# violetamenendez/zest-nerf

Measured on AMD Instinct MI355X. Metric: rendered rays/sec (1024-ray x 128-sample batch per GPU), higher is better.
Workload: dtype bf16; 1 GPU; nsff_static_1024x128; rays_per_gpu=1024, samples_per_ray=128, rays_total=1024, collective=none, ranks=1, backend=none

## Files before the change

### zest-nerf_amd/csrc/fused.cuh

```cuda
#pragma once
#include "mlp_engine.cuh"
#include "zest_sample_ops.cuh"

namespace zest {

constexpr int kMaxViews = 16;
constexpr int kCamStride = 24;

struct FusedNet {
    const float *bias;
    const uint4 *tiles;
    const float4 *vol;
    const float4 *imgs;
    const float *w2cs, *intr;
    int D, Hv, Wv, V, H, W;
    int head, v2;
};

struct FusedArgs {
    const float *ndc, *pts, *z, *dir;
    int R, S;
    FusedNet st, dy;
    float frame_idx;
    int white_bkgd;
    int bpr;
    float *partials;
    float *out;
    unsigned long long *stamps;
    int ray_ranges;
};

struct RayState {
    float Ts = 1.f, Tb = 1.f, Tf = 1.f;
    float s[5] = {0, 0, 0, 0, 0}, bl[5] = {0, 0, 0, 0, 0}, fg[4] = {0, 0, 0, 0};
    __device__ __forceinline__ void chain(const float *p, bool dyn) {
#pragma unroll
        for (int i = 0; i < 5; i++) s[i] += Ts * p[1 + i];
        Ts *= p[0];
        if (dyn) {
#pragma unroll
            for (int i = 0; i < 5; i++) bl[i] += Tb * p[7 + i];
            Tb *= p[6];
#pragma unroll
            for (int i = 0; i < 4; i++) fg[i] += Tf * p[13 + i];
            Tf *= p[12];
        }
    }
    __device__ __forceinline__ void emit(int white_bkgd, float *__restrict__ out_row) const {
        float4 *o = reinterpret_cast<float4 *>(out_row);
        const float bg = white_bkgd ? 1.0f - s[4] : 0.0f;
        o[0] = make_float4(s[0] + bg, s[1] + bg, s[2] + bg, s[3]);
        o[1] = make_float4(s[4], bl[0], bl[1], bl[2]);
        o[2] = make_float4(bl[3], fg[0], fg[1], fg[2]);
        float zero = 0.f;
        asm volatile("" : "+v"(zero));
        o[3] = make_float4(fg[3], bl[4], zero, zero);
    }
    __device__ __forceinline__ void save(float *c) const {
        c[0] = Ts, c[1] = Tb, c[2] = Tf;
#pragma unroll
        for (int i = 0; i < 5; i++) c[3 + i] = s[i], c[8 + i] = bl[i];
#pragma unroll
        for (int i = 0; i < 4; i++) c[13 + i] = fg[i];
    }
    __device__ __forceinline__ void load(const float *c) {
        Ts = c[0], Tb = c[1], Tf = c[2];
#pragma unroll
        for (int i = 0; i < 5; i++) s[i] = c[3 + i], bl[i] = c[8 + i];
#pragma unroll
        for (int i = 0; i < 4; i++) fg[i] = c[13 + i];
    }
};
constexpr int kCarryFloats = 20;

template <class Rec>
__device__ __forceinline__ void combine_ray(Rec rec, int bpr, bool dyn, int white_bkgd, float *__restrict__ out_row) {
    RayState st;
    for (int b = 0; b < bpr; b++) st.chain(rec(b), dyn);
    st.emit(white_bkgd, out_row);
}

template <int EP, int C, int L, int NK>
__device__ __forceinline__ void encode_pe_operand(const float (&x)[4], int grp, OpArr<NK, ep_parts(EP)> &op) {
    static_assert((L / 2) * C + 1 <= NK * 8 && L % 2 == 0, "position layout");
    const float quarter = (grp & 1) ? 0.25f : 0.0f;
    const float gscale = (grp & 2) ? 2.0f * 0.15915494309189535f : 0.15915494309189535f;
    const float gband = (grp & 2) ? 2.0f : 1.0f;
    float rev[C];
#pragma unroll
    for (int c = 0; c < C; c++) rev[c] = x[c] * gscale;
    const float raw = grp == 0 ? x[0] : (grp == 1 ? x[1] : (grp == 2 ? x[2] : (C > 3 ? x[3] : 0.0f)));
#pragma unroll
    for (int t = 0; t < NK; t++) {
        float v[8];
#pragma unroll
        for (int e = 0; e < 8; e++) {
            const int m = 8 * t + e;
            if (m < (L / 2) * C) {
                if constexpr (EP == ZEST_PREC_F16X3) {
                    float sn, cs;
                    zest_sincos(x[m % C] * (gband * (float)(1 << (2 * (m / C)))), &sn, &cs);
                    v[e] = (grp & 1) ? cs : sn;
                } else {
                    const float r = fmaf(rev[m % C], (float)(1 << (2 * (m / C))), quarter);
                    v[e] = __builtin_amdgcn_sinf(__builtin_amdgcn_fractf(r));
                }
            } else if (m == (L / 2) * C) {
                v[e] = raw;
            } else {
                v[e] = 0.0f;
            }
        }
        store_tile<EP>(v, op, t);
    }
}

__device__ __forceinline__ float4 zest_color_tap_fast(const float4 *__restrict__ img, int H, int W,
                                                      const float *__restrict__ P, float px, float py, float pz) {
    const float4 r0 = *reinterpret_cast<const float4 *>(P), r1 = *reinterpret_cast<const float4 *>(P + 4),
                 r2 = *reinterpret_cast<const float4 *>(P + 8);
    const float qx = fmaf(pz, r0.z, fmaf(py, r0.y, fmaf(px, r0.x, r0.w)));
    const float qy = fmaf(pz, r1.z, fmaf(py, r1.y, fmaf(px, r1.x, r1.w)));
    const float qz = fmaf(pz, r2.z, fmaf(py, r2.y, fmaf(px, r2.x, r2.w)));
    const float rz = __builtin_amdgcn_rcpf(qz);
    float fx = qx * rz, fy = qy * rz;
    const float wm = (float)(W - 1), hm = (float)(H - 1);
    const float mask = (fx > 0.0f && fx < wm && fy > 0.0f && fy < hm) ? 1.0f : 0.0f;
    fx = fminf(fmaxf(fx, 0.0f), wm), fy = fminf(fmaxf(fy, 0.0f), hm);
    const float x0f = floorf(fx), y0f = floorf(fy);
    const float tx = fx - x0f, ty = fy - y0f;
    const int x0 = (int)x0f, y0 = (int)y0f;
    const int i00 = y0 * W + x0, dx = x0 + 1 < W ? 1 : 0, dy = y0 + 1 < H ? W : 0;
#ifdef ZEST_EXPERIMENT_TAP_SAME
    const float4 a = img[i00 & 0], b = img[(i00 + dx) & 0], d = img[(i00 + dy) & 0], e = img[(i00 + dy + dx) & 0];
#else
    const float4 a = img[i00], b = img[i00 + dx], d = img[i00 + dy], e = img[i00 + dy + dx];
#endif
    const float w00 = (1.0f - tx) * (1.0f - ty), w10 = tx * (1.0f - ty), w01 = (1.0f - tx) * ty, w11 = tx * ty;
    float4 o;
    o.x = fmaf(w11, e.x, fmaf(w01, d.x, fmaf(w10, b.x, w00 * a.x)));
    o.y = fmaf(w11, e.y, fmaf(w01, d.y, fmaf(w10, b.y, w00 * a.y)));
    o.z = fmaf(w11, e.z, fmaf(w01, d.z, fmaf(w10, b.z, w00 * a.z)));
    o.w = mask;
    return o;
}

template <int EP, int NK>
__device__ __forceinline__ void encode_feat_operand(const FusedNet &n, const float *cams_lds,
                                                    const float (&ndc)[4], const float (&pw)[3],
                                                    int grp, bool valid, OpArr<NK, ep_parts(EP)> &op) {
    float v[NK * 8];
#pragma unroll
    for (int i = 0; i < NK * 8; i++) v[i] = 0.0f;
    auto view_tap = [&](int view, float *dst) {
        const int vc = view < n.V ? view : n.V - 1;
        const float *cl = cams_lds + vc * kCamStride;
        float4 o;
        if constexpr (EP == ZEST_PREC_F16X3) {
            ZestCam cam;
#pragma unroll
            for (int i = 0; i < 3; i++) {
#pragma unroll
                for (int j = 0; j < 4; j++) cam.r[i][j] = cl[4 * i + j];
#pragma unroll
                for (int j = 0; j < 3; j++) cam.k[i][j] = cl[12 + 3 * i + j];
            }
#ifdef ZEST_EXPERIMENT_TAP_SAME
            o = zest_color_tap<true>(n.imgs, n.H, n.W, cam, pw[0], pw[1], pw[2]);
#else
            o = zest_color_tap(n.imgs + (size_t)vc * n.H * n.W, n.H, n.W, cam, pw[0], pw[1], pw[2]);
#endif
        } else {
            o = zest_color_tap_fast(n.imgs + vc * (n.H * n.W), n.H, n.W, cl, pw[0], pw[1], pw[2]);
        }
        const bool on = view < n.V;
        dst[0] = on ? o.x : 0.f, dst[1] = on ? o.y : 0.f, dst[2] = on ? o.z : 0.f, dst[3] = on ? o.w : 0.f;
    };
#ifdef ZEST_EXPERIMENT_NO_GATHER
    valid = false;
#endif
#ifdef ZEST_EXPERIMENT_FAKE_FEAT
    if (valid) {
#pragma unroll
        for (int i = 0; i < NK * 8; i++)
            v[i] = __builtin_amdgcn_fractf(ndc[0] * (13.37f + (float)i) + ndc[2] * 7.1f + (float)grp * 0.31f) - 0.25f;
    }
    valid = false;
#endif
    const int rv = feat_volume_round(n.V);
    if (valid) {
        float vv[4] = {0.f, 0.f, 0.f, 0.f};
        if (grp < 2) {
            float fx = zest_unnorm(ndc[0], n.Wv), fy = zest_unnorm(ndc[1], n.Hv), fz = zest_unnorm(ndc[2], n.D);
            fx = fminf(fmaxf(fx, -2.0f), (float)n.Wv + 1.0f);
            fy = fminf(fmaxf(fy, -2.0f), (float)n.Hv + 1.0f);
            fz = fminf(fmaxf(fz, -2.0f), (float)n.D + 1.0f);
            const float x0f = floorf(fx), y0f = floorf(fy), z0f = floorf(fz);
            const float tx = fx - x0f, ty = fy - y0f, tz = fz - z0f;
            const int x0 = (int)x0f, y0 = (int)y0f, z0 = (int)z0f;
            float4 tap[8];
            float wgt[8];
#pragma unroll
            for (int c = 0; c < 8; c++) {
                const int dx = c & 1, dy = (c >> 1) & 1, dz = c >> 2;
                const int xi = x0 + dx, yi = y0 + dy, zi = z0 + dz;
                const bool ok = (unsigned)xi < (unsigned)n.Wv && (unsigned)yi < (unsigned)n.Hv &&
                                (unsigned)zi < (unsigned)n.D;
                const int xc = min(max(xi, 0), n.Wv - 1), yc = min(max(yi, 0), n.Hv - 1),
                          zc = min(max(zi, 0), n.D - 1);
                wgt[c] = ok ? (dx ? tx : 1.0f - tx) * (dy ? ty : 1.0f - ty) * (dz ? tz : 1.0f - tz) : 0.0f;
#ifdef ZEST_EXPERIMENT_TAP_SAME
                tap[c] = n.vol[(((yc * n.Wv + xc) * n.D + zc) & 0) + grp];
#else
                tap[c] = n.vol[2 * ((yc * n.Wv + xc) * n.D + zc) + grp];
#endif
            }
#pragma unroll
            for (int c = 0; c < 8; c++) {
                vv[0] = fmaf(wgt[c], tap[c].x, vv[0]), vv[1] = fmaf(wgt[c], tap[c].y, vv[1]);
                vv[2] = fmaf(wgt[c], tap[c].z, vv[2]), vv[3] = fmaf(wgt[c], tap[c].w, vv[3]);
            }
        }
#pragma unroll
        for (int r = 0; r < 2 * NK; r++) {
            float *dst = v + 8 * (r >> 1) + 4 * (r & 1);
            if (r < rv) {
                view_tap(4 * r + grp, dst);
            } else if (r == rv) {
                if (n.V > 4 * rv) view_tap(grp >= 2 ? 4 * rv + grp - 2 : n.V, dst);
                if (grp < 2) dst[0] = vv[0], dst[1] = vv[1], dst[2] = vv[2], dst[3] = vv[3];
            }
        }
    }
#pragma unroll
    for (int t = 0; t < NK; t++) {
        float w8[8];
#pragma unroll
        for (int e = 0; e < 8; e++) w8[e] = v[8 * t + e];
        store_tile<EP>(w8, op, t);
    }
}

template <bool PROJ>
__device__ __forceinline__ void stage_cams(const FusedNet &n, float *lds) {
    if (!n.w2cs) return;
    const int nv = n.imgs ? n.V : 1;
    for (int i = threadIdx.x; i < nv * kCamStride; i += blockDim.x) {
        const int v = i / kCamStride, k = i % kCamStride;
        float val = 0.0f;
        if constexpr (PROJ) {
            if (k < 12 && n.intr) {
                const int row = k >> 2, col = k & 3;
                const float *K = n.intr + 9 * v + 3 * row, *Rt = n.w2cs + 16 * v + col;
                val = fmaf(K[2], Rt[8], fmaf(K[1], Rt[4], K[0] * Rt[0]));
            } else if (k >= 12) {
                val = n.w2cs[16 * v + (k - 12)];
            }
        } else {
            if (k < 12) val = n.w2cs[16 * v + k];
            else if (k < 21 && n.intr) val = n.intr[9 * v + (k - 12)];
        }
        lds[i] = val;
    }
}

#ifndef ZEST_FUSED_WAVES
#define ZEST_FUSED_WAVES 8
#endif
constexpr int kFusedWaves = ZEST_FUSED_WAVES;
constexpr int kPartialFloats = 20;
constexpr int fused_cb(int EP) { return EP == ZEST_PREC_F16X3 ? 1 : 2; }

struct BlockSamples {
    float x[4], pw[3], zz, dist;
    bool valid;
};

template <int BS>
__device__ __forceinline__ float block_sum(float v) {
    if constexpr (BS == 32) return lower_half_sum(v);
    v += dpp_f<0xB1>(0.f, v);
    v += dpp_f<0x4E>(0.f, v);
    v += dpp_f<0x141>(0.f, v);
    v += dpp_f<0x140>(0.f, v);
    return readlane_f<0>(v);
}
template <int BS>
__device__ __forceinline__ float block_excl_prod(float f, int c, float *total) {
    if constexpr (BS == 32) return lower_half_excl_prod(f, c, total);
    float v = f;
    v *= dpp_f<0x111>(1.f, v);
    v *= dpp_f<0x112>(1.f, v);
    v *= dpp_f<0x114>(1.f, v);
    v *= dpp_f<0x118>(1.f, v);
    *total = readlane_f<15>(v);
    const float ex = dpp_f<0x138>(1.f, v);
    return c == 0 ? 1.0f : ex;
}

#ifndef ZEST_FUSED_WG_PER_CU
#define ZEST_FUSED_WG_PER_CU 1
#endif
#ifndef ZEST_REBUILD_PTS
#define ZEST_REBUILD_PTS 0
#endif
#ifndef ZEST_GATHER_FENCE
#define ZEST_GATHER_FENCE 1
#endif
#ifndef ZEST_EARLY_DYN_GATHER
#define ZEST_EARLY_DYN_GATHER 0
#endif
template <int EP, int NT_FEAT_S, bool DYN, int NT_FEAT_D, bool V2S = false>
__global__ __launch_bounds__(kFusedWaves * 64, kFusedWaves * ZEST_FUSED_WG_PER_CU / 4) void fused_blocks_kernel(FusedArgs a) {
    constexpr bool MOD_S = NT_FEAT_S > 0, MOD_D = NT_FEAT_D > 0;
    constexpr int NP = ep_parts(EP), CB = fused_cb(EP), BS = 16 * CB;
    if constexpr (EP == ZEST_PREC_F16) engine_fp16_overflow_clamp();
    constexpr int UNITS_S = stream_units(4, NT_FEAT_S, NP), UNITS_D = DYN ? stream_units(6, NT_FEAT_D, NP) : 0;
    using Ring = RingTiles<kFusedWaves, UNITS_S, UNITS_D>;
    constexpr int kFdBytes = (DYN && MOD_D && ZEST_EARLY_DYN_GATHER) ? kFusedWaves * CB * (NT_FEAT_D / 2) * NP * 1024 : 0;
    constexpr int kStBytes = DYN ? kFusedWaves * 32 * 24 : 0;
    constexpr bool kMc = mcache_for(EP, MOD_S, NT_FEAT_S / 2) || (DYN && mcache_for(EP, MOD_D, NT_FEAT_D / 2));
    constexpr int kMcWaveBytes = kMc ? kMcJB * CB * 1024 : 0;
    __shared__ __attribute__((aligned(16))) char lds[kRingUnits * 1024 + 2 * kMaxViews * kCamStride * 4 +
                                                     kFusedWaves * 32 * 8 + 2 * kSlots * 4 +
                                                     kFusedWaves * kPartialFloats * 4 + kFusedWaves * 32 * 16 +
                                                     kFdBytes + kStBytes + 2 * kCarryFloats * 4 +
                                                     kFusedWaves * kMcWaveBytes];
    static_assert(sizeof(lds) <= 163840, "LDS budget of one workgroup per CU");
    static_assert((sizeof(lds) - kFusedWaves * kMcWaveBytes) % 16 == 0, "the modulation cache starts 16-byte aligned");
    float *cams_s = reinterpret_cast<float *>(lds + kRingUnits * 1024), *cams_d = cams_s + kMaxViews * kCamStride;
    float2 *zd_lds = reinterpret_cast<float2 *>(cams_d + kMaxViews * kCamStride);
    constexpr bool PROJ = EP != ZEST_PREC_F16X3;
    stage_cams<PROJ>(a.st, cams_s);
    if (DYN) stage_cams<PROJ>(a.dy, cams_d);
    int *ring_flags = reinterpret_cast<int *>(zd_lds + kFusedWaves * 32);
    float *rec_lds = reinterpret_cast<float *>(ring_flags + 2 * kSlots);
    float4 *x_lds = reinterpret_cast<float4 *>(rec_lds + kFusedWaves * kPartialFloats);
    uint4 *fd_lds = reinterpret_cast<uint4 *>(x_lds + kFusedWaves * 32);
    float2 *st_lds = reinterpret_cast<float2 *>(reinterpret_cast<char *>(fd_lds) + kFdBytes);
    float *carry_lds = reinterpret_cast<float *>(reinterpret_cast<char *>(st_lds) + kStBytes);
    char *mc_lds = lds + sizeof(lds) - kFusedWaves * kMcWaveBytes;
#ifdef ZEST_RING_FLAGS
    Ring::init_flags(ring_flags);
#endif
    __syncthreads();

    const int lane0 = threadIdx.x & 63;
    const int wave = __builtin_amdgcn_readfirstlane(threadIdx.x >> 6);
    const Ring tiles{lds, (gptr_u4)a.st.tiles, (gptr_u4)a.dy.tiles, lane0, lane0 >> 4, wave,
                     (unsigned)(wave * Ring::kPieces * 64 + lane0) * 16u,
                     (unsigned)(uintptr_t)(__attribute__((address_space(3))) char *)lds +
                         (unsigned)wave * Ring::kPieces * 1024u
#ifdef ZEST_RING_FLAGS
                     , (unsigned)(uintptr_t)(__attribute__((address_space(3))) char *)ring_flags
#endif
    };
    tiles.init_addr();
    if constexpr (kMc)
        tiles.init_mcache((unsigned)(uintptr_t)(__attribute__((address_space(3))) char *)mc_lds +
                          (unsigned)wave * kMcWaveBytes + (unsigned)lane0 * 16u);
    tiles.prologue();

    const bool ranges = a.ray_ranges != 0;
    const int n_wg = (int)gridDim.x;
#ifndef ZEST_NO_XCD_ORDER
    const int wg = n_wg % 8 == 0 ? (int)(blockIdx.x % 8) * (n_wg / 8) + (int)(blockIdx.x / 8) : (int)blockIdx.x;
#else
    const int wg = (int)blockIdx.x;
#endif
    int range_b0, range_nb;
    if (ranges) {
        range_b0 = (int)((long long)wg * a.R / n_wg) * a.bpr;
        range_nb = (int)((long long)(wg + 1) * a.R / n_wg) * a.bpr - range_b0;
    } else {
        const int n_blocks = a.R * a.bpr;
        const int share = ((n_blocks + kFusedWaves - 1) / kFusedWaves + n_wg - 1) / n_wg * kFusedWaves;
        range_b0 = wg * share, range_nb = min(share, n_blocks - range_b0);
    }
    auto block_of = [&](int pass) {
        const int lb = pass * kFusedWaves + wave;
        return __builtin_amdgcn_readfirstlane(lb < range_nb ? range_b0 + lb : -1);
    };
    auto fetch = [&](int g, int cb, int col, BlockSamples &b) {
        const int r = g >= 0 ? g / a.bpr : 0, s = (g >= 0 ? g % a.bpr : 0) * BS + 16 * cb + col;
        b.valid = g >= 0 && s < a.S;
        b.x[0] = b.x[1] = b.x[2] = 0.f, b.x[3] = a.frame_idx;
        b.pw[0] = b.pw[1] = b.pw[2] = 0.f, b.zz = 0.f, b.dist = 0.f;
        const float *dir = a.dir + 3 * r;
        if (b.valid) {
            const size_t m = (size_t)r * a.S + s;
            const float *zr = a.z + (size_t)r * a.S;
            b.x[0] = a.ndc[3 * m], b.x[1] = a.ndc[3 * m + 1], b.x[2] = a.ndc[3 * m + 2];
            if (a.pts) b.pw[0] = a.pts[3 * m], b.pw[1] = a.pts[3 * m + 1], b.pw[2] = a.pts[3 * m + 2];
            b.zz = zr[s];
            const float dnorm = sqrtf(dir[0] * dir[0] + dir[1] * dir[1] + dir[2] * dir[2]);
            b.dist = ((s + 1 < a.S) ? (zr[s + 1] - b.zz) : 1e10f) * dnorm;
        }
    };
    auto join = [](const f32x4 (&t)[CB], int i) {
        if constexpr (CB == 1) {
            return t[0][i];
        } else {
            const auto r = __builtin_amdgcn_permlane16_swap(__float_as_uint(t[0][i]), __float_as_uint(t[CB - 1][i]), false, false);
            return __uint_as_float(r[0]);
        }
    };
#ifdef ZEST_STAMPS
    unsigned long long st_enc = 0, st_eng = 0, st_comp = 0, st_n = 0;
    const unsigned long long st_t0 = __builtin_amdgcn_s_memtime(), st_r0 = __builtin_amdgcn_s_memrealtime();
#define ZEST_STAMP(var) do { const unsigned long long t_ = __builtin_amdgcn_s_memtime(); var += t_ - st_last; st_last = t_; } while (0)
#else
#define ZEST_STAMP(var) do {} while (0)
#endif
    for (int k = 0; k * kFusedWaves < range_nb; k++) {
        const int pass = k;
#ifdef ZEST_STAMPS
        unsigned long long st_last = __builtin_amdgcn_s_memtime();
        st_n++;
#endif
        const int g = block_of(pass);
        if (__builtin_expect(g < 0, 0)) {
            tiles.finish(0, UNITS_S + UNITS_D);
        } else {
        int lane = lane0;
        asm volatile("" : "+v"(lane));
        const int col = lane & 15, grp = lane >> 4, cbs = lane & (BS - 1);
        int unit = 0;
        f32x4 head_s[CB], rgb_s[CB], head_d[CB], rgb_d[CB];
        auto views_of = [&](const FusedNet &n, const float *cams) {
            return [&, cams](OpArr<1, NP> (&views)[CB]) {
                const float *dir = a.dir + 3 * (g >= 0 ? g / a.bpr : 0);
                float dv[4] = {0.f, 0.f, 0.f, 0.f};
                zest_view_dir(dir, n.w2cs ? cams + (PROJ ? 12 : 0) : nullptr, dv);
                encode_pe_operand<EP, 3, 4, 1>(dv, grp, views[0]);
#pragma unroll
                for (int cb = 1; cb < CB; cb++) views[cb] = views[0];
            };
        };
        OpArr<NT_FEAT_S / 2, NP> feat_s[CB];
#pragma unroll
        for (int cb = 0; cb < CB; cb++) {
            BlockSamples b;
            fetch(g, cb, col, b);
            if (grp == 0) {
                zd_lds[wave * 32 + 16 * cb + col] = make_float2(b.zz, b.valid ? b.dist : -1.0f);
                x_lds[wave * 32 + 16 * cb + col] = make_float4(b.x[0], b.x[1], b.x[2], 0.0f);
            }
            if constexpr (MOD_S) encode_feat_operand<EP, NT_FEAT_S / 2>(a.st, cams_s, b.x, b.pw, grp, b.valid, feat_s[cb]);
#if ZEST_GATHER_FENCE
            if constexpr (DYN && NT_FEAT_S >= 4) __builtin_amdgcn_sched_barrier(0);
#endif
            if constexpr (DYN && MOD_D && ZEST_EARLY_DYN_GATHER) {
                OpArr<NT_FEAT_D / 2, NP> fd;
                encode_feat_operand<EP, NT_FEAT_D / 2>(a.dy, cams_d, b.x, b.pw, grp, b.valid, fd);
#pragma unroll
                for (int t = 0; t < NT_FEAT_D / 2; t++)
#pragma unroll
                    for (int pt = 0; pt < NP; pt++)
                        fd_lds[(((wave * CB + cb) * (NT_FEAT_D / 2) + t) * NP + pt) * 64 + lane] =
                            __builtin_bit_cast(uint4, fd.t[pt][t]);
            }
        }
        auto pts_static = [&](OpArr<2, NP> (&o)[CB], int token) __attribute__((always_inline)) {
#pragma unroll
            for (int cb = 0; cb < CB; cb++) {
                int at = wave * 32 + 16 * cb + col;
                asm volatile("" : "+v"(at) : "v"(token));
                const float4 xv = x_lds[at];
                const float x4[4] = {xv.x, xv.y, xv.z, 0.0f};
#ifdef ZEST_EXPERIMENT_NO_ENCODE
#pragma unroll
                for (int t = 0; t < 2; t++) o[cb].t[0][t] = bf16x8{(short)lane, 1, 2, 3, 4, 5, 6, 7};
#else
                encode_pe_operand<EP, 3, 10, 2>(x4, grp, o[cb]);
#endif
            }
        };
        auto pts_dynamic = [&](OpArr<3, NP> (&o)[CB], int token) __attribute__((always_inline)) {
#pragma unroll
            for (int cb = 0; cb < CB; cb++) {
                int at = wave * 32 + 16 * cb + col;
                asm volatile("" : "+v"(at) : "v"(token));
                const float4 xv = x_lds[at];
                const float x4[4] = {xv.x, xv.y, xv.z, a.frame_idx};
                encode_pe_operand<EP, 4, 10, 3>(x4, grp, o[cb]);
            }
        };
        ZEST_STAMP(st_enc);
        if constexpr (ZEST_REBUILD_PTS) {
            engine_forward<EP, CB, 4, MOD_S, NT_FEAT_S, V2S, true>(tiles, unit, pts_static, feat_s,
                                                        views_of(a.st, cams_s), head_s, rgb_s);
        } else {
            OpArr<2, NP> pts_keep[CB];
            pts_static(pts_keep, 0);
            auto pts_copy = [&](OpArr<2, NP> (&o)[CB], int) __attribute__((always_inline)) {
#pragma unroll
                for (int cb = 0; cb < CB; cb++) o[cb] = pts_keep[cb];
            };
            engine_forward<EP, CB, 4, MOD_S, NT_FEAT_S, V2S, true>(tiles, unit, pts_copy, feat_s,
                                                        views_of(a.st, cams_s), head_s, rgb_s);
        }
        ZEST_STAMP(st_eng);
        float rec[kPartialFloats];
#pragma unroll
        for (int i = 0; i < kPartialFloats; i++) rec[i] = 0.f;
        float zz, dist, cr, cg, cb, al_s;
        bool valid;
        {
            const float2 zd = zd_lds[wave * 32 + cbs];
            zz = zd.x, dist = fmaxf(zd.y, 0.0f), valid = zd.y >= 0.0f;
            float sg = join(head_s, 0);
            cr = join(rgb_s, 0), cg = join(rgb_s, 1), cb = join(rgb_s, 2);
            if (V2S) {
                cr = zest_sigmoid(cr), cg = zest_sigmoid(cg), cb = zest_sigmoid(cb), sg = fmaxf(sg, 0.f);
            }
            cr = zest_sigmoid(cr), cg = zest_sigmoid(cg), cb = zest_sigmoid(cb);
            al_s = valid ? 1.0f - expf(-fmaxf(sg, 0.f) * dist) : 0.0f;
            float tot;
            const float w = al_s * block_excl_prod<BS>(1.0f - al_s + 1e-10f, cbs, &tot);
            rec[0] = tot;
            rec[1] = block_sum<BS>(w * cr), rec[2] = block_sum<BS>(w * cg), rec[3] = block_sum<BS>(w * cb);
            rec[4] = block_sum<BS>(w * zz), rec[5] = block_sum<BS>(w);
        }
        if (DYN) {
            const float blend_s = zest_sigmoid(join(head_s, 1));
            if (lane < BS) {
                st_lds[(wave * 3 + 0) * 32 + lane] = make_float2(cr, cg);
                st_lds[(wave * 3 + 1) * 32 + lane] = make_float2(cb, al_s);
                st_lds[(wave * 3 + 2) * 32 + lane] = make_float2(blend_s, 0.0f);
            }
            OpArr<NT_FEAT_D / 2, NP> feat_d[CB];
            if constexpr (MOD_D && ZEST_EARLY_DYN_GATHER) {
#pragma unroll
                for (int cbi = 0; cbi < CB; cbi++)
#pragma unroll
                    for (int t = 0; t < NT_FEAT_D / 2; t++)
#pragma unroll
                        for (int pt = 0; pt < NP; pt++)
                            feat_d[cbi].t[pt][t] = __builtin_bit_cast(
                                bf16x8, fd_lds[(((wave * CB + cbi) * (NT_FEAT_D / 2) + t) * NP + pt) * 64 + lane]);
            } else if constexpr (MOD_D) {
#pragma unroll
                for (int cbi = 0; cbi < CB; cbi++) {
                    BlockSamples b;
                    fetch(g, cbi, col, b);
                    encode_feat_operand<EP, NT_FEAT_D / 2>(a.dy, cams_d, b.x, b.pw, grp, b.valid, feat_d[cbi]);
                }
            }
            ZEST_STAMP(st_comp);
            if constexpr (ZEST_REBUILD_PTS) {
                engine_forward<EP, CB, 6, MOD_D, NT_FEAT_D, false, true>(tiles, unit, pts_dynamic, feat_d,
                                                            views_of(a.dy, cams_d), head_d, rgb_d);
            } else {
                OpArr<3, NP> pts_keep[CB];
                pts_dynamic(pts_keep, 0);
                auto pts_copy = [&](OpArr<3, NP> (&o)[CB], int) __attribute__((always_inline)) {
#pragma unroll
                    for (int cb = 0; cb < CB; cb++) o[cb] = pts_keep[cb];
                };
                engine_forward<EP, CB, 6, MOD_D, NT_FEAT_D, false, true>(tiles, unit, pts_copy, feat_d,
                                                            views_of(a.dy, cams_d), head_d, rgb_d);
            }
            ZEST_STAMP(st_eng);
            const float2 s0 = st_lds[(wave * 3 + 0) * 32 + cbs], s1 = st_lds[(wave * 3 + 1) * 32 + cbs],
                         s2 = st_lds[(wave * 3 + 2) * 32 + cbs];
            cr = s0.x, cg = s0.y, cb = s1.x, al_s = s1.y;
            const float blend = s2.x;
            const float er = zest_sigmoid(join(rgb_d, 0)), eg = zest_sigmoid(join(rgb_d, 1)),
                        eb = zest_sigmoid(join(rgb_d, 2));
            const float sg_d = join(head_d, 0);
            const float a_fg = valid ? 1.0f - expf(-fmaxf(sg_d, 0.f) * dist) : 0.0f;
            const float a_d = a_fg * blend, a_st = al_s * (1.0f - blend);
            float tot_b, tot_f;
            const float Tb = block_excl_prod<BS>((1.0f - a_d) * (1.0f - a_st) + 1e-10f, cbs, &tot_b);
            const float wf = a_fg * block_excl_prod<BS>(1.0f - a_fg + 1e-10f, cbs, &tot_f);
            const float wd = Tb * a_d, ws = Tb * a_st;
            rec[6] = tot_b;
            rec[7] = block_sum<BS>(wd * er + ws * cr), rec[8] = block_sum<BS>(wd * eg + ws * cg);
            rec[9] = block_sum<BS>(wd * eb + ws * cb), rec[10] = block_sum<BS>((wd + ws) * zz);
            rec[11] = block_sum<BS>(wd);
            rec[12] = tot_f;
            rec[13] = block_sum<BS>(wf * er), rec[14] = block_sum<BS>(wf * eg), rec[15] = block_sum<BS>(wf * eb);
            rec[16] = block_sum<BS>(wf * zz);
        }
        if (lane == 0 && g >= 0) {
            float4 *o = ranges ? reinterpret_cast<float4 *>(rec_lds + wave * kPartialFloats)
                               : reinterpret_cast<float4 *>(a.partials + (size_t)g * kPartialFloats);
#pragma unroll
            for (int i = 0; i < (DYN ? 5 : 2); i++)
                o[i] = make_float4(rec[4 * i], rec[4 * i + 1], rec[4 * i + 2], rec[4 * i + 3]);
        }
        }
#ifdef ZEST_EXPERIMENT_NO_FINISH
        if (false) {
#else
        if (ranges) {
#endif
            __syncthreads();
            const int rb = g >= 0 ? g % a.bpr : 0;
            if (lane0 == 0 && g >= 0 && (wave == 0 || rb == 0)) {
                RayState st;
                if (rb != 0) st.load(carry_lds + ((k + 1) & 1) * kCarryFloats);
                const int n = min(a.bpr - rb, kFusedWaves - wave);
                for (int b = 0; b < n; b++) st.chain(rec_lds + (wave + b) * kPartialFloats, DYN);
                if (rb + n == a.bpr) st.emit(a.white_bkgd, a.out + (size_t)(g / a.bpr) * 16);
                else st.save(carry_lds + (k & 1) * kCarryFloats);
            }
        }
        ZEST_STAMP(st_comp);
        tiles.next_pass();
    }
    tiles.drain();
#ifdef ZEST_RING_FLAGS
    if (tiles.poisoned && lane0 == 0) {
        a.partials[0] = __builtin_nanf("");
    }
#endif
#ifdef ZEST_STAMPS
    if (a.stamps && lane0 == 0) {
        unsigned long long *o = a.stamps + (size_t)(blockIdx.x * kFusedWaves + wave) * 8;
        o[0] = __builtin_amdgcn_s_memtime() - st_t0, o[1] = st_enc, o[2] = st_eng, o[3] = st_comp;
        o[4] = tiles.t_wait, o[5] = tiles.t_issue, o[6] = __builtin_amdgcn_s_memrealtime() - st_r0,
        o[7] = st_n | (tiles.t_vm << 16);
    }
#endif
}

#define ZEST_FUSED_VARIANT(ptag, EP, tag, NTS, DYN, NTD, V2S) ZEST_FUSED_VARIANT_(ptag, EP, tag, NTS, DYN, NTD, V2S)
#define ZEST_FUSED_VARIANT_(ptag, EP, tag, NTS, DYN, NTD, V2S)                                   \
    int fused_launch_##ptag##_##tag(const FusedArgs &a, int blocks, hipStream_t stream) {        \
        hipLaunchKernelGGL((fused_blocks_kernel<EP, NTS, DYN, NTD, V2S>), dim3(blocks),          \
                           dim3(kFusedWaves * 64), 0, stream, a);                                \
        ZEST_RETURN_LAUNCH("zest_render_fused_fwd(" #ptag "_" #tag ")");                         \
    }                                                                                            \
    int fused_units_##ptag##_##tag(int which) {                                                  \
        return which == 0 ? stream_units(4, NTS, ep_parts(EP)) : (DYN ? stream_units(6, NTD, ep_parts(EP)) : 0); \
    }

#define ZEST_FUSED_DECL1(ptag, tag)                                                     \
    int fused_launch_##ptag##_##tag(const FusedArgs &a, int blocks, hipStream_t stream); \
    int fused_units_##ptag##_##tag(int which);
#define ZEST_FUSED_DECL(tag) ZEST_FUSED_DECL1(bf16, tag) ZEST_FUSED_DECL1(f16, tag) ZEST_FUSED_DECL1(x3, tag)
ZEST_FUSED_DECL(s0)
ZEST_FUSED_DECL(s2)
ZEST_FUSED_DECL(s4)
ZEST_FUSED_DECL(s0d0)
ZEST_FUSED_DECL(s2d0)
ZEST_FUSED_DECL(s4d0)
ZEST_FUSED_DECL(s2d2)
ZEST_FUSED_DECL(s4d2)
ZEST_FUSED_DECL(s2v)
ZEST_FUSED_DECL(s4v)

}
```

### zest-nerf_amd/csrc/fused.hip

```cpp
#include <string.h>
#include "fused.cuh"
#include "mlp_plan.h"

namespace zest {

__global__ void fused_combine_kernel(const float *__restrict__ partials, int R, int bpr, int dyn,
                                     int white_bkgd, float *__restrict__ out) {
    const int r = blockIdx.x * blockDim.x + threadIdx.x;
    if (r >= R) return;
    combine_ray([&](int b) { return partials + ((size_t)r * bpr + b) * kPartialFloats; }, bpr, dyn != 0,
                white_bkgd, out + (size_t)r * 16);
}

}

namespace {

bool fill_net(const zest_mlp_desc *d, const void *packed, const zest_view_set *vs, int pts_ch, int precision,
              zest::FusedNet *n, int *nt_feat, int *units, const char **err) {
    memset(n, 0, sizeof(*n));
    if (!d || !packed) return *err = "descriptor and packed weights are required", false;
    if (d->in_ch_pts != pts_ch) return *err = "unexpected in_ch_pts for this slot", false;
    if (d->net_type != 0 && d->net_type != 2) return *err = "net_type must be 0 ('v0') or 2 ('v2')", false;
    zest::MlpPlan plan;
    if (!zest::build_plan(*d, precision, zest::ORDER_ACC, &plan, err, false)) return false;
    n->bias = (const float *)packed;
    n->tiles = (const uint4 *)((const char *)packed + plan.bias_bytes);
    n->head = d->head, n->v2 = d->net_type == 2;
    *nt_feat = d->use_feat ? plan.nt_feat : 0;
    *units = plan.n_tiles;
    if (((uintptr_t)packed & 15) != 0) return *err = "packed weights must be 16-byte aligned", false;
    if (vs) {
        n->w2cs = vs->w2cs, n->intr = vs->intrinsics;
        n->vol = (const float4 *)vs->vol_cl, n->imgs = (const float4 *)vs->imgs_cl;
        n->D = vs->D, n->Hv = vs->Hv, n->Wv = vs->Wv, n->V = vs->V, n->H = vs->H, n->W = vs->W;
    }
    if (d->use_feat) {
        if (!vs || !vs->vol_cl || !vs->imgs_cl || !vs->w2cs || !vs->intrinsics)
            return *err = "a net with features needs volume, images and cameras", false;
        if (vs->D < 1 || vs->Hv < 1 || vs->Wv < 1 || vs->H < 2 || vs->W < 2)
            return *err = "bad volume / image shape", false;
        if ((long long)vs->D * vs->Hv * vs->Wv >= (1LL << 30))
            return *err = "volume too large for the fused kernel's 32-bit voxel indices (2^30 voxels)", false;
        if (vs->V < 1 || vs->V > zest::kMaxViews || 8 + 4 * vs->V != d->in_ch_feat)
            return *err = "view count does not match in_ch_feat = 8 + 4V", false;
        if (((uintptr_t)vs->vol_cl | (uintptr_t)vs->imgs_cl) & 15)
            return *err = "volume / images must be 16-byte aligned", false;
    } else {
        n->vol = nullptr, n->imgs = nullptr;
    }
    return true;
}

}

#ifdef ZEST_STAMPS
constexpr size_t kStampBytes = 1024 * 8 * 8 * 8;
#else
constexpr size_t kStampBytes = 0;
#endif

static int g_pass_shape = 0;

extern "C" int zest_render_fused_set_passes(int shape) {
    ZEST_CHECK_ARG(shape >= 0 && shape <= 2,
                   "zest_render_fused_set_passes: shape must be 0 (auto), 1 (dense: equal block shares) or 2 (ray ranges)");
    g_pass_shape = shape;
    return 0;
}

extern "C" int zest_render_fused_pass_shape(int R, int S, int precision, int cus, int *ray_ranges, int *n_wg,
                                            int *rounds) {
    ZEST_CHECK_ARG(R >= 0 && S >= 1 && zest::prec_is_engine(precision) && ray_ranges,
                   "zest_render_fused_pass_shape: bad argument");
    if (cus <= 0) {
        int dev = 0;
        if (hipGetDevice(&dev) != hipSuccess ||
            hipDeviceGetAttribute(&cus, hipDeviceAttributeMultiprocessorCount, dev) != hipSuccess)
            cus = 256;
    }
    const int bs = 16 * zest::fused_cb(precision), bpr = (S + bs - 1) / bs;
    const int W = zest::kFusedWaves;
    const int P = zest_div_up((long long)R * bpr, W), G0 = P < cus ? P : cus;
    const int dense_rounds = G0 ? zest_div_up(P, G0) : 0, dense_wg = G0 ? zest_div_up(P, dense_rounds) : 0;
    const int n = R < cus ? R : cus;
    const int range_rounds = n ? zest_div_up((long long)zest_div_up(R, n) * bpr, W) : 0;
    int take = range_rounds <= dense_rounds ? 1 : 0;
    if (g_pass_shape == 1) take = 0;
    if (g_pass_shape == 2) take = 1;
    *ray_ranges = take;
    if (n_wg) *n_wg = take ? n : dense_wg;
    if (rounds) *rounds = take ? range_rounds : dense_rounds;
    return 0;
}

extern "C" size_t zest_render_fused_workspace(int R, int S) {
    if (R <= 0 || S <= 0) return 16 + kStampBytes;
    return (size_t)R * ((S + 15) / 16) * zest::kPartialFloats * sizeof(float) + kStampBytes;
}

extern "C" int zest_render_fused_fwd(const float *ndc, const float *pts, const float *z,
                                     const float *rays_dir, int R, int S,
                                     const zest_mlp_desc *desc_static, const void *packed_static,
                                     const zest_view_set *views_static,
                                     const zest_mlp_desc *desc_dynamic, const void *packed_dynamic,
                                     const zest_view_set *views_dynamic, float frame_idx,
                                     int precision, int white_bkgd, void *workspace, float *out,
                                     void *stream) {
    if (R == 0) return 0;
    ZEST_CHECK_ARG(ndc && z && rays_dir && out && workspace,
                   "zest_render_fused_fwd: ndc, z, rays_dir, workspace, out required");
    ZEST_CHECK_ARG(((uintptr_t)workspace & 15) == 0, "zest_render_fused_fwd: workspace must be 16-byte aligned");
    ZEST_CHECK_ARG(R >= 0 && S >= 1, "zest_render_fused_fwd: bad shape R=%d S=%d", R, S);
    ZEST_CHECK_ARG(zest::prec_is_engine(precision),
                   "zest_render_fused_fwd: precision must be ZEST_PREC_BF16, _F16 or _F16X3 (the exact-product "
                   "fp32 kernel exists per operator only: zest_mlp_fwd)");
    ZEST_CHECK_ARG(((uintptr_t)out & 15) == 0, "zest_render_fused_fwd: out must be 16-byte aligned");
    zest::FusedArgs a;
    memset(&a, 0, sizeof(a));
    a.ndc = ndc, a.pts = pts, a.z = z, a.dir = rays_dir, a.R = R, a.S = S;
    a.frame_idx = frame_idx, a.white_bkgd = white_bkgd, a.out = out;
    const int bs = 16 * zest::fused_cb(precision);
    a.bpr = (S + bs - 1) / bs, a.partials = (float *)workspace;
#ifdef ZEST_STAMPS
    a.stamps = (unsigned long long *)((char *)workspace + zest_render_fused_workspace(R, S) - kStampBytes);
#endif
    const char *err = nullptr;
    int nts = 0, ntd = 0, units_s = 0, units_d = 0;
    ZEST_CHECK_ARG(fill_net(desc_static, packed_static, views_static, 63, precision, &a.st, &nts, &units_s, &err),
                   "zest_render_fused_fwd: static net: %s", err);
    const bool dyn = desc_dynamic != nullptr;
    if (dyn) {
        ZEST_CHECK_ARG(fill_net(desc_dynamic, packed_dynamic, views_dynamic, 84, precision, &a.dy, &ntd, &units_d, &err),
                       "zest_render_fused_fwd: dynamic net: %s", err);
        ZEST_CHECK_ARG(desc_static->head == ZEST_HEAD_BLEND && desc_dynamic->head == ZEST_HEAD_DYNAMIC,
                       "zest_render_fused_fwd: blending needs a static net with the blend head and "
                       "a dynamic net with the scene-flow heads");
    }
    ZEST_CHECK_ARG(pts || (!a.st.vol && !a.dy.vol), "zest_render_fused_fwd: pts required with features");
    if (R == 0) return 0;
    int dev = 0, cus = 256;
    if (hipGetDevice(&dev) != hipSuccess ||
        hipDeviceGetAttribute(&cus, hipDeviceAttributeMultiprocessorCount, dev) != hipSuccess)
        cus = 256;
    int blocks = 0;
    zest_render_fused_pass_shape(R, S, precision, cus, &a.ray_ranges, &blocks, nullptr);
    hipStream_t st = (hipStream_t)stream;
    const bool v2s = a.st.v2 != 0;
    ZEST_CHECK_ARG(!(v2s && (dyn || nts == 0)),
                   "zest_render_fused_fwd: a 'v2' net is rendered by the single-net kernels with features only");
    const int key = (v2s ? 1000 : 0) + (dyn ? 100 : 0) + nts * 10 + ntd;
    int rc = -1;
#define ZEST_CASE1(ptag, tag)                                                                    \
    ZEST_CHECK_ARG(zest::fused_units_##ptag##_##tag(0) == units_s && zest::fused_units_##ptag##_##tag(1) == units_d, \
                   "zest_render_fused_fwd: packed stream is %d+%d units, kernel expects %d+%d",  \
                   units_s, units_d, zest::fused_units_##ptag##_##tag(0), zest::fused_units_##ptag##_##tag(1)); \
    rc = zest::fused_launch_##ptag##_##tag(a, blocks, st);
#define ZEST_CASE(k, tag)                                                                        \
    case k:                                                                                      \
        if (precision == ZEST_PREC_BF16) { ZEST_CASE1(bf16, tag) }                               \
        else if (precision == ZEST_PREC_F16) { ZEST_CASE1(f16, tag) }                            \
        else { ZEST_CASE1(x3, tag) }                                                             \
        break;
    switch (key) {
        ZEST_CASE(0, s0)
        ZEST_CASE(20, s2)
        ZEST_CASE(40, s4)
        ZEST_CASE(100, s0d0)
        ZEST_CASE(120, s2d0)
        ZEST_CASE(140, s4d0)
        ZEST_CASE(122, s2d2)
        ZEST_CASE(142, s4d2)
        ZEST_CASE(1020, s2v)
        ZEST_CASE(1040, s4v)
        default:
            zest_set_error("zest_render_fused_fwd: no fused variant for %d static / %d dynamic feature "
                           "tiles%s", nts, ntd, dyn ? "" : " (static only)");
            return (int)hipErrorInvalidValue;
    }
#undef ZEST_CASE
#undef ZEST_CASE1
    if (rc != 0 || a.ray_ranges) return rc;
    hipLaunchKernelGGL(zest::fused_combine_kernel, dim3(zest_div_up(R, 128)), dim3(128), 0, st,
                       a.partials, R, a.bpr, dyn ? 1 : 0, white_bkgd, out);
    ZEST_RETURN_LAUNCH("zest_render_fused_fwd(combine)");
}
```

### zest-nerf_amd/csrc/mlp.hip

```cpp
#include <string.h>
#include <map>
#include <mutex>
#include <tuple>
#include "mlp_plan.h"
#include "zest_common.cuh"
#include "mlp_engine.cuh"

namespace {

using zest::MlpPlan;

struct DevPlan {
    MlpPlan plan;
    uint32_t *tile_src = nullptr, *bias_src = nullptr, *hdr_src = nullptr;
    uint8_t *unit_part = nullptr;
};

std::mutex g_mu;
std::map<std::tuple<int, int, int, int, int, int, int, int, int, int, int, int>, DevPlan *> g_plans;

constexpr int kOrderBwd = 99;

DevPlan *get_plan(const zest_mlp_desc &d, int precision, int order, bool need_tables) {
    int dev = 0;
    if (hipGetDevice(&dev) != hipSuccess) dev = 0;
    std::lock_guard<std::mutex> lk(g_mu);
    auto key = std::make_tuple(d.in_ch_pts, d.use_feat ? d.in_ch_feat : 0, d.in_ch_views,
                               d.use_feat, d.net_type, d.head, precision, order, d.depth, d.width, d.skip_mask, dev);
    auto it = g_plans.find(key);
    DevPlan *dp = it == g_plans.end() ? nullptr : it->second;
    if (!dp) {
        dp = new DevPlan();
        const char *err = nullptr;
        const bool ok = order == kOrderBwd ? zest::build_bwd_plan(d, &dp->plan, &err)
                                           : zest::build_plan(d, precision, order, &dp->plan, &err);
        if (!ok) {
            zest_set_error("MLP shape not supported: %s", err);
            delete dp;
            return nullptr;
        }
        g_plans[key] = dp;
    }
    if (need_tables && !dp->tile_src) {
        const size_t nt = dp->plan.tile_src.size() * 4, nb = dp->plan.bias_src.size() * 4;
        const size_t nh = dp->plan.hdr_src.size() * 4, np = dp->plan.unit_part.size();
        hipError_t e = hipMalloc(&dp->tile_src, nt);
        if (e == hipSuccess) e = hipMalloc(&dp->unit_part, np ? np : 4);
        if (e == hipSuccess && np) e = hipMemcpy(dp->unit_part, dp->plan.unit_part.data(), np, hipMemcpyHostToDevice);
        if (e == hipSuccess) e = hipMalloc(&dp->bias_src, nb ? nb : 4);
        if (e == hipSuccess) e = hipMalloc(&dp->hdr_src, nh ? nh : 4);
        if (e == hipSuccess) e = hipMemcpy(dp->tile_src, dp->plan.tile_src.data(), nt, hipMemcpyHostToDevice);
        if (e == hipSuccess && nb) e = hipMemcpy(dp->bias_src, dp->plan.bias_src.data(), nb, hipMemcpyHostToDevice);
        if (e == hipSuccess && nh) e = hipMemcpy(dp->hdr_src, dp->plan.hdr_src.data(), nh, hipMemcpyHostToDevice);
        if (e != hipSuccess) {
            zest_set_error("zest_mlp_pack: uploading gather tables: %s", hipGetErrorString(e));
            dp->tile_src = nullptr;
            return nullptr;
        }
    }
    return dp;
}

inline int order_for(int precision) {
    return zest::prec_is_engine(precision) ? zest::ORDER_ACC : zest::ORDER_NATURAL;
}

struct ParamTable {
    const float *p[2 * ZEST_P_COUNT];
};

template <int PREC>
__global__ void pack_kernel(ParamTable pt, const uint32_t *__restrict__ tile_src, size_t n_w,
                            const uint32_t *__restrict__ bias_src, size_t n_b,
                            const uint8_t *__restrict__ unit_part,
                            float *__restrict__ bias_out, void *__restrict__ w_out) {
    const size_t i = (size_t)blockIdx.x * blockDim.x + threadIdx.x;
    if (i < n_b) {
        const uint32_t s = bias_src[i];
        bias_out[i] = s == 0xFFFFFFFFu ? 0.0f : pt.p[2 * (s >> 24) + 1][s & 0xFFFFFF];
    }
    if (i < n_w) {
        const uint32_t s = tile_src[i];
        const float v = s == 0xFFFFFFFFu ? 0.0f : pt.p[2 * (s >> 24)][s & 0xFFFFFF];
        if (PREC == ZEST_PREC_BF16) {
            ((__hip_bfloat16 *)w_out)[i] = __float2bfloat16(v);
        } else if (PREC == ZEST_PREC_F16) {
            ((_Float16 *)w_out)[i] = (_Float16)v;
        } else if (PREC == ZEST_PREC_F16X3) {
            const _Float16 hi = (_Float16)v;
            ((_Float16 *)w_out)[i] = unit_part[i / 512] ? (_Float16)((v - (float)hi) * 2048.0f) : hi;
        } else {
            ((float *)w_out)[i] = v;
        }
    }
}

__global__ void pack_headers_kernel(ParamTable pt, const uint32_t *__restrict__ hdr_src, size_t n,
                                    char *__restrict__ w_out) {
    const size_t i = (size_t)blockIdx.x * blockDim.x + threadIdx.x;
    if (i >= n) return;
    const uint32_t s = hdr_src[i];
    if (s == 0xFFFFFFFFu) return;
    const size_t unit = i / 64, j = i % 64;
    ((float *)(w_out + unit * 1024))[j] = pt.p[2 * (s >> 24) + 1][s & 0xFFFFFF];
}

struct F32Op {
    int njb, nseg, kind0, nt0, kind1, nt1, mod, relu, tile_base, tiles_per_jb, bias_block;
    int src_h, dst;
};
struct F32Prog {
    F32Op op[zest::kNumOps];
    int n_ops, W;
    int P, F, Vw, C_in, C_out, nt_feat, net_v2, act_out, head;
    int rows_pts, rows_feat;
};

constexpr int kF32Samples = 32;

__global__ __launch_bounds__(256, 1) void mlp_f32_kernel(F32Prog pr, const float *__restrict__ bias,
                                                         const float4 *__restrict__ tiles,
                                                         const float *__restrict__ x, int M,
                                                         float *__restrict__ out) {
    extern __shared__ __attribute__((aligned(16))) float smem[];
    float *b_pts = smem;
    float *b_feat = b_pts + pr.rows_pts * 32;
    float *b_views = b_feat + pr.rows_feat * 32;
    float *b_h[2] = {b_views + 32 * 32, b_views + 32 * 32 + pr.W * 32};
    const int tid = threadIdx.x, lane = tid & 63, wave = tid >> 6;
    const int col = lane & 31, half = lane >> 5;
    const int n_in_rows = pr.rows_pts + pr.rows_feat + 32;

    for (int m0 = blockIdx.x * kF32Samples; m0 < M; m0 += gridDim.x * kF32Samples) {
        __syncthreads();
        for (int i = tid; i < n_in_rows * 32; i += 256) smem[i] = 0.0f;
        __syncthreads();
        const int nvalid = min(kF32Samples, M - m0);
        for (int i = tid; i < nvalid * pr.C_in; i += 256) {
            const int s = i / pr.C_in, c = i % pr.C_in;
            const float v = x[(size_t)m0 * pr.C_in + i];
            float *dst = c < pr.P ? b_pts + c * 32
                                  : (c < pr.P + pr.F ? b_feat + (c - pr.P) * 32
                                                     : b_views + (c - pr.P - pr.F) * 32);
            dst[s] = v;
        }
        __syncthreads();
#pragma unroll 1
        for (int o = 0; o < pr.n_ops; o++) {
            const F32Op op = pr.op[o];
            for (int jb = wave; jb < op.njb; jb += 4) {
                const float4 *tp = tiles + ((size_t)op.tile_base + (size_t)jb * op.tiles_per_jb) * 64 + lane;
                f32x16 acc, macc;
                {
                    const float *bb = bias + (size_t)(op.bias_block + jb) * 32 + half * 16;
#pragma unroll
                    for (int i = 0; i < 16; i++) acc[i] = bb[i];
                }
                if (op.mod) {
                    const float *mb = bias + (size_t)jb * 32 + half * 16;
#pragma unroll
                    for (int i = 0; i < 16; i++) macc[i] = mb[i];
                    for (int t = 0; t < pr.nt_feat; t++, tp += 64) {
                        const float4 a = *tp;
                        const float *bp = b_feat + (t * 8 + 4 * half) * 32 + col;
                        macc = __builtin_amdgcn_mfma_f32_32x32x2f32(a.x, bp[0], macc, 0, 0, 0);
                        macc = __builtin_amdgcn_mfma_f32_32x32x2f32(a.y, bp[32], macc, 0, 0, 0);
                        macc = __builtin_amdgcn_mfma_f32_32x32x2f32(a.z, bp[64], macc, 0, 0, 0);
                        macc = __builtin_amdgcn_mfma_f32_32x32x2f32(a.w, bp[96], macc, 0, 0, 0);
                    }
                }
                for (int sg = 0; sg < op.nseg; sg++) {
                    const int kind = sg ? op.kind1 : op.kind0, nt = sg ? op.nt1 : op.nt0;
                    const float *src = kind == zest::SEG_PTS ? b_pts
                                       : kind == zest::SEG_VIEWS ? b_views : b_h[op.src_h];
                    for (int t = 0; t < nt; t++, tp += 64) {
                        const float4 a = *tp;
                        const float *bp = src + (t * 8 + 4 * half) * 32 + col;
                        acc = __builtin_amdgcn_mfma_f32_32x32x2f32(a.x, bp[0], acc, 0, 0, 0);
                        acc = __builtin_amdgcn_mfma_f32_32x32x2f32(a.y, bp[32], acc, 0, 0, 0);
                        acc = __builtin_amdgcn_mfma_f32_32x32x2f32(a.z, bp[64], acc, 0, 0, 0);
                        acc = __builtin_amdgcn_mfma_f32_32x32x2f32(a.w, bp[96], acc, 0, 0, 0);
                    }
                }
#pragma unroll
                for (int i = 0; i < 16; i++) {
                    const int row = 32 * jb + (i & 3) + 8 * (i >> 2) + 4 * half;
                    float v = acc[i];
                    if (op.mod) v = pr.net_v2 ? v + macc[i] : v * macc[i];
                    if (op.relu) v = fmaxf(v, 0.0f);
                    if (op.dst < 2) {
                        b_h[op.dst][row * 32 + col] = v;
                    } else if (col < nvalid) {
                        float *orow = out + (size_t)(m0 + col) * pr.C_out;
                        if (o == pr.n_ops - 1) {
                            if (row < 3) orow[row] = pr.act_out ? zest_sigmoid(v) : v;
                        } else if (row == 0) {
                            orow[3] = pr.act_out ? fmaxf(v, 0.0f) : v;
                        } else if (3 + row < pr.C_out) {
                            const bool is_sf = pr.head == ZEST_HEAD_DYNAMIC && row <= 6;
                            orow[3 + row] = is_sf ? tanhf(v) : zest_sigmoid(v);
                        }
                    }
                }
            }
            __syncthreads();
        }
    }
}

F32Prog make_f32_prog(const MlpPlan &p) {
    F32Prog pr = {};
    const int D = p.shape.D, t = (D - 1) & 1;
    pr.n_ops = p.n_ops, pr.W = p.shape.W;
    for (int o = 0; o < p.n_ops; o++) {
        const zest::OpPlan &s = p.op[o];
        F32Op &d = pr.op[o];
        const int src_h = o < D ? (o + 1) & 1 : (o == D + 2 ? 1 - t : t);
        const int dst = o < D ? o & 1 : (o == D + 1 ? 1 - t : (o == D + 2 ? t : 2));
        d.njb = s.njb, d.nseg = s.nseg, d.kind0 = s.seg[0].kind, d.nt0 = s.seg[0].ntiles;
        d.kind1 = s.seg[1].kind, d.nt1 = s.seg[1].ntiles, d.mod = s.mod, d.relu = s.relu;
        d.tile_base = s.tile_base, d.tiles_per_jb = s.tiles_per_jb, d.bias_block = s.bias_block;
        d.src_h = src_h, d.dst = dst;
    }
    pr.P = p.desc.in_ch_pts, pr.F = p.desc.use_feat ? p.desc.in_ch_feat : 0, pr.Vw = p.desc.in_ch_views;
    pr.C_in = pr.P + pr.F + pr.Vw;
    pr.C_out = p.desc.head == ZEST_HEAD_NONE ? 4 : (p.desc.head == ZEST_HEAD_BLEND ? 5 : 12);
    pr.nt_feat = p.nt_feat, pr.net_v2 = p.desc.net_type >= 2, pr.act_out = p.desc.net_type == 2, pr.head = p.desc.head;
    pr.rows_pts = p.nt_pts * 8, pr.rows_feat = p.nt_feat * 8;
    return pr;
}

}

namespace zest {
size_t bwd_stream_bytes(const zest_mlp_desc &d) {
    DevPlan *dp = get_plan(d, ZEST_PREC_BF16, kOrderBwd, false);
    return dp ? dp->plan.bytes : 0;
}
int bwd_stream_units_of(const zest_mlp_desc &d) {
    DevPlan *dp = get_plan(d, ZEST_PREC_BF16, kOrderBwd, false);
    return dp ? dp->plan.tail_unit0 : -1;
}
int pack_bwd_stream(const zest_mlp_desc &d, const float *const *params, void *packed, hipStream_t stream) {
    DevPlan *dp = get_plan(d, ZEST_PREC_BF16, kOrderBwd, true);
    if (!dp) return (int)hipErrorInvalidValue;
    const MlpPlan &p = dp->plan;
    ParamTable pt;
    for (int i = 0; i < 2 * ZEST_P_COUNT; i++) pt.p[i] = params[i];
    const size_t n_w = p.tile_src.size(), n_h = p.hdr_src.size();
    hipLaunchKernelGGL(pack_kernel<ZEST_PREC_BF16>, dim3(zest_div_up(n_w, 256)), dim3(256), 0, stream, pt, dp->tile_src,
                       n_w, dp->bias_src, (size_t)0, dp->unit_part, (float *)packed, packed);
    hipLaunchKernelGGL(pack_headers_kernel, dim3(zest_div_up(n_h, 256)), dim3(256), 0, stream, pt, dp->hdr_src, n_h,
                       (char *)packed);
    ZEST_RETURN_LAUNCH("zest_mlp_train16_pack");
}
}

extern "C" size_t zest_mlp_packed_bytes(const zest_mlp_desc *desc, int precision) {
    if (!desc) return 0;
    DevPlan *dp = get_plan(*desc, precision, order_for(precision), false);
    return dp ? dp->plan.bytes : 0;
}

extern "C" int zest_mlp_pack(const zest_mlp_desc *desc, int precision, const float *const *params,
                             void *packed, void *stream) {
    ZEST_CHECK_ARG(desc && params && packed, "zest_mlp_pack: null argument");
    DevPlan *dp = get_plan(*desc, precision, order_for(precision), true);
    if (!dp) return (int)hipErrorInvalidValue;
    const MlpPlan &p = dp->plan;
    ParamTable pt;
    for (int i = 0; i < 2 * ZEST_P_COUNT; i++) pt.p[i] = params[i];
    bool need[ZEST_P_COUNT] = {};
    for (int i = 0; i < p.shape.D; i++) need[i] = true;
    need[ZEST_P_PTS_BIAS] = desc->use_feat != 0;
    need[ZEST_P_VIEWS] = need[ZEST_P_FEATURE] = need[ZEST_P_ALPHA] = need[ZEST_P_RGB] = true;
    need[ZEST_P_HEAD0] = desc->head != ZEST_HEAD_NONE;
    need[ZEST_P_HEAD1] = desc->head == ZEST_HEAD_DYNAMIC;
    for (int i = 0; i < ZEST_P_COUNT; i++)
        ZEST_CHECK_ARG(!need[i] || (params[2 * i] && params[2 * i + 1]),
                       "zest_mlp_pack: parameter slot %d (weight and bias) is required", i);
    ZEST_CHECK_ARG(((uintptr_t)packed & 15) == 0, "zest_mlp_pack: packed must be 16-byte aligned");
    const size_t n_w = p.tile_src.size(), n_b = p.bias_src.size();
    const size_t n = n_w > n_b ? n_w : n_b;
    void *w_out = (char *)packed + p.bias_bytes;
#define ZEST_PACK(PREC)                                                                            \
    hipLaunchKernelGGL(pack_kernel<PREC>, dim3(zest_div_up(n, 256)), dim3(256), 0, (hipStream_t)stream, \
                       pt, dp->tile_src, n_w, dp->bias_src, n_b, dp->unit_part, (float *)packed, w_out)
    if (zest::prec_is_engine(precision)) {
        if (precision == ZEST_PREC_BF16) ZEST_PACK(ZEST_PREC_BF16);
        else if (precision == ZEST_PREC_F16) ZEST_PACK(ZEST_PREC_F16);
        else ZEST_PACK(ZEST_PREC_F16X3);
        const size_t n_h = p.hdr_src.size();
        if (n_h)
            hipLaunchKernelGGL(pack_headers_kernel, dim3(zest_div_up(n_h, 256)), dim3(256), 0,
                               (hipStream_t)stream, pt, dp->hdr_src, n_h, (char *)w_out);
    } else {
        ZEST_PACK(ZEST_PREC_F32);
    }
#undef ZEST_PACK
    ZEST_RETURN_LAUNCH("zest_mlp_pack");
}

extern "C" int zest_mlp_fwd(const zest_mlp_desc *desc, int precision, const void *packed,
                            const float *x, int M, float *out, void *stream) {
    if (M == 0) return 0;
    ZEST_CHECK_ARG(desc && packed && x && out, "zest_mlp_fwd: null argument");
    ZEST_CHECK_ARG(M >= 0, "zest_mlp_fwd: M=%d", M);
    DevPlan *dp = get_plan(*desc, precision, order_for(precision), false);
    if (!dp) return (int)hipErrorInvalidValue;
    if (M == 0) return 0;
    const MlpPlan &p = dp->plan;
    const float *bias = (const float *)packed;
    const void *tiles = (const char *)packed + p.bias_bytes;
    if (precision == ZEST_PREC_F32) {
        const F32Prog pr = make_f32_prog(p);
        const size_t lds = (size_t)(pr.rows_pts + pr.rows_feat + 32 + 2 * pr.W) * 32 * sizeof(float);
        const int blocks = zest_div_up(M, kF32Samples);
        hipLaunchKernelGGL(mlp_f32_kernel, dim3(blocks < 4096 ? blocks : 4096), dim3(256), lds,
                           (hipStream_t)stream, pr, bias, (const float4 *)tiles, x, M, out);
        ZEST_RETURN_LAUNCH("zest_mlp_fwd(f32)");
    }
    return zest::mlp_engine_launch(p, tiles, x, M, out, (hipStream_t)stream);
}
```

### zest-nerf_amd/csrc/mlp_engine.cuh

```cuda
#pragma once
#include <hip/hip_bf16.h>
#include "mlp_plan.h"
#include "zest_common.cuh"

typedef __attribute__((ext_vector_type(16))) float f32x16;
typedef __attribute__((ext_vector_type(4))) float f32x4;
typedef __attribute__((ext_vector_type(8))) short bf16x8;
typedef __attribute__((ext_vector_type(4))) float v4f;
typedef __attribute__((ext_vector_type(4))) unsigned v4u;
typedef const __attribute__((address_space(1))) v4u *gptr_u4;
typedef __attribute__((address_space(3))) int lds_int;

namespace zest {

constexpr int stream_units_raw(int nt_pts, int nt_feat, int parts = 1) {
    const int mod = nt_feat * parts, P = nt_pts * parts, H = 16 * parts;
    return 8 * (1 + mod + P) + 6 * 8 * (1 + mod + H) + 8 * (1 + mod + P + H)
           + (1 + H) + 8 * (1 + H) + 4 * (1 + H + 2 * parts) + (1 + H / 2);
}
constexpr int stream_units(int nt_pts, int nt_feat, int parts = 1) {
    return (stream_units_raw(nt_pts, nt_feat, parts) + kStreamAlign - 1) / kStreamAlign * kStreamAlign;
}

#ifndef ZEST_CHUNK
#define ZEST_CHUNK 16
#define ZEST_SLOTS 8
#define ZEST_AHEAD 4
#endif
constexpr int kChunk = ZEST_CHUNK, kSlots = ZEST_SLOTS, kRingUnits = kChunk * kSlots, kAhead = ZEST_AHEAD;
static_assert(kStreamAlign % kRingUnits == 0, "stream padding must be a multiple of the ring size");
static_assert(kSlots >= kAhead + 1, "a slot is refilled while the previous chunk may still be read");

#ifndef ZEST_DEFER_DMA
#define ZEST_DEFER_DMA 0
#endif
#ifndef ZEST_ISSUERS
#define ZEST_ISSUERS 8
#endif
template <int NW, int UNITS_A, int UNITS_B>
struct RingTiles {
    static constexpr int kIssuers = ZEST_ISSUERS < NW ? ZEST_ISSUERS : NW;
    static constexpr int kPieces = kChunk / kIssuers;
    static constexpr int kChunksA = UNITS_A / kChunk, kChunks = (UNITS_A + UNITS_B) / kChunk;
    static_assert(kChunk % kIssuers == 0 && UNITS_A % kRingUnits == 0 && UNITS_B % kRingUnits == 0, "");
    char *ring;
    gptr_u4 src_a, src_b;
    int lane, grp, wave;
    unsigned voff;
    unsigned lds_wave_base;
#ifdef ZEST_RING_FLAGS
    unsigned flags;
    mutable int gen_base = 0;
    mutable int poisoned = 0;
#endif
#ifdef ZEST_STAMPS
    mutable unsigned long long t_wait = 0, t_issue = 0, t_vm = 0;
#endif

    __device__ __forceinline__ void issue(int chunk) const {
        if (kIssuers < NW && wave >= kIssuers) return;
        const int c = chunk % kChunks;
        unsigned off = (unsigned)((c < kChunksA ? c : c - kChunksA) * kChunk * 1024);
        asm volatile("" : "+s"(off));
        const __attribute__((address_space(1))) char *sb =
            (const __attribute__((address_space(1))) char *)(c < kChunksA ? src_a : src_b) + off;
        const unsigned dst = lds_wave_base + (c % kSlots) * kChunk * 1024;
        static_assert(kPieces == 1 || kPieces == 2 || kPieces == 4, "pieces per wave");
        if (kPieces == 1)
            asm volatile("s_mov_b32 m0, %2\n\ts_nop 0\n\tglobal_load_lds_dwordx4 %0, %1"
                         :: "v"(voff), "s"(sb), "s"(dst) : "memory", "m0");
        else if (kPieces == 2)
            asm volatile("s_mov_b32 m0, %2\n\ts_nop 0\n\tglobal_load_lds_dwordx4 %0, %1\n\t"
                         "global_load_lds_dwordx4 %0, %1 offset:1024"
                         :: "v"(voff), "s"(sb), "s"(dst) : "memory", "m0");
        else
            asm volatile("s_mov_b32 m0, %2\n\ts_nop 0\n\tglobal_load_lds_dwordx4 %0, %1\n\t"
                         "global_load_lds_dwordx4 %0, %1 offset:1024\n\t"
                         "global_load_lds_dwordx4 %0, %1 offset:2048\n\t"
                         "global_load_lds_dwordx4 %0, %1 offset:3072"
                         :: "v"(voff), "s"(sb), "s"(dst) : "memory", "m0");
    }
#ifdef ZEST_RING_FLAGS
    static_assert(kSlots >= kAhead + 2, "flag ring: a slot is refilled while laggards read its neighbours");
    static constexpr int off_landed(int slot) { return 8 * (slot % kSlots); }
    static constexpr int off_done(int slot) { return 8 * ((slot % kSlots - kAhead + kSlots) % kSlots) + 4; }
    static __device__ void init_flags(int *f) {
        if (threadIdx.x < 2 * kSlots) f[threadIdx.x] = 0;
        __syncthreads();
        if (threadIdx.x == 0) f[off_done(kSlots - 1) / 4] = -NW;
    }
    template <int OFF_A, int OFF_B>
    __device__ __forceinline__ void bump2() const {
        unsigned long long save;
        asm volatile("s_mov_b64 %0, exec\n\ts_mov_b64 exec, 1\n\t"
                     "ds_add_u32 %2, %1 offset:%3\n\tds_add_u32 %2, %1 offset:%4\n\ts_mov_b64 exec, %0"
                     : "=&s"(save) : "v"(1u), "v"(flags), "i"(OFF_A), "i"(OFF_B) : "memory");
    }
    __device__ __forceinline__ void prologue() const {
#pragma unroll
        for (int c = 0; c < kAhead; c++) issue(c);
        asm volatile("s_waitcnt vmcnt(%0)" ::"i"((kAhead - 1) * kPieces) : "memory");
        unsigned long long save;
        asm volatile("s_mov_b64 %0, exec\n\ts_mov_b64 exec, 1\n\t"
                     "ds_add_u32 %2, %1 offset:%3\n\ts_mov_b64 exec, %0"
                     : "=&s"(save) : "v"(1u), "v"(flags), "i"(off_landed(0)) : "memory");
    }
    __device__ __forceinline__ void next_pass() const { gen_base += kChunks / kSlots; }
    static constexpr int kPreRead = 5;
    typedef int v2i __attribute__((ext_vector_type(2)));
    mutable v2i flag_pre = {0, 0};
    __device__ __forceinline__ void pre_read(int chunk) const {
        flag_pre = *(const volatile __attribute__((address_space(3))) v2i *)(flags + off_landed(chunk));
    }
    template <int OFF>
    __device__ __forceinline__ void await(int need_l, int need_d) const {
        unsigned va = (unsigned)flag_pre.x, vb = (unsigned)flag_pre.y;
        int sa, sb, tries = 1 << 14;
        asm volatile("0:\n\t"
                     "v_readfirstlane_b32 %2, %0\n\t"
                     "v_readfirstlane_b32 %3, %1\n\t"
                     "s_nop 1\n\t"
                     "s_cmp_ge_i32 %2, %6\n\t"
                     "s_cselect_b32 %2, 1, 0\n\t"
                     "s_cmp_ge_i32 %3, %7\n\t"
                     "s_cselect_b32 %3, 1, 0\n\t"
                     "s_and_b32 %2, %2, %3\n\t"
                     "s_cbranch_scc1 1f\n\t"
                     "s_sub_u32 %4, %4, 1\n\t"
                     "s_cmp_eq_u32 %4, 0\n\t"
                     "s_cbranch_scc1 1f\n\t"
                     "s_sleep 1\n\t"
                     "ds_read_b32 %0, %5 offset:%8\n\t"
                     "ds_read_b32 %1, %5 offset:%9\n\t"
                     "s_waitcnt lgkmcnt(0)\n\t"
                     "s_branch 0b\n\t"
                     "1:"
                     : "+v"(va), "+v"(vb), "=&s"(sa), "=&s"(sb), "+s"(tries)
                     : "v"(flags), "s"(need_l), "s"(need_d), "i"(OFF), "i"(OFF + 4)
                     : "memory", "scc");
        if (tries == 0) poisoned = 1;
    }
    __device__ __forceinline__ void enter_chunk(int chunk) const {
#ifdef ZEST_STAMPS
        const unsigned long long t0 = __builtin_amdgcn_s_memtime();
#endif
        asm volatile("s_waitcnt vmcnt(%0)" ::"i"((kAhead - 2) * kPieces) : "memory");
#ifdef ZEST_STAMPS
        t_vm += __builtin_amdgcn_s_memtime() - t0;
#endif
        const int need_l = NW * (gen_base + chunk / kSlots + 1), need_d = NW * (gen_base + (chunk + kAhead) / kSlots);
        if (chunk % kChunks == 0) pre_read(chunk);
        switch (chunk % kSlots) {
#define ZEST_CASE(S) case S: bump2<off_landed(S + 1), off_done(S + kSlots - 1)>(); await<off_landed(S)>(need_l, need_d); break;
            ZEST_CASE(0) ZEST_CASE(1) ZEST_CASE(2) ZEST_CASE(3) ZEST_CASE(4) ZEST_CASE(5) ZEST_CASE(6) ZEST_CASE(7)
            ZEST_CASE(8) ZEST_CASE(9) ZEST_CASE(10) ZEST_CASE(11) ZEST_CASE(12) ZEST_CASE(13) ZEST_CASE(14) ZEST_CASE(15)
#undef ZEST_CASE
        }
        static_assert(kSlots <= 16, "extend the slot switch");
#ifdef ZEST_STAMPS
        const unsigned long long t1 = __builtin_amdgcn_s_memtime();
#endif
        issue(chunk + kAhead);
#ifdef ZEST_STAMPS
        t_wait += t1 - t0, t_issue += __builtin_amdgcn_s_memtime() - t1;
#endif
    }
#else
    __device__ __forceinline__ void prologue() const {
#pragma unroll
        for (int c = 0; c < kAhead; c++) issue(c);
    }
    __device__ __forceinline__ void next_pass() const {}
    __device__ __forceinline__ void enter_chunk(int chunk) const {
#ifdef ZEST_STAMPS
        const unsigned long long t0 = __builtin_amdgcn_s_memtime();
#endif
        flush();
        asm volatile("s_waitcnt vmcnt(%0)" ::"i"((kAhead - 1) * kPieces) : "memory");
#ifdef ZEST_STAMPS
        t_vm += __builtin_amdgcn_s_memtime() - t0;
#endif
#ifndef ZEST_EXPERIMENT_NO_BARRIER
        __builtin_amdgcn_s_barrier();
#endif
        asm volatile("" ::: "memory");
#ifdef ZEST_STAMPS
        const unsigned long long t1 = __builtin_amdgcn_s_memtime();
#endif
#ifndef ZEST_EXPERIMENT_NO_DMA
#if ZEST_DEFER_DMA
        pending = chunk + kAhead;
#else
        issue(chunk + kAhead);
#endif
#endif
#ifdef ZEST_STAMPS
        t_wait += t1 - t0, t_issue += __builtin_amdgcn_s_memtime() - t1;
#endif
    }
#endif
    mutable int pending = -1;
    __device__ __forceinline__ void flush() const {
#if ZEST_DEFER_DMA
#ifdef ZEST_STAMPS
        const unsigned long long t1 = __builtin_amdgcn_s_memtime();
#endif
        if (pending >= 0) issue(pending);
        pending = -1;
#ifdef ZEST_STAMPS
        t_issue += __builtin_amdgcn_s_memtime() - t1;
#endif
#endif
    }
    __device__ __forceinline__ void touch(int unit) const {
        if (unit % kChunk == 0) enter_chunk(unit / kChunk);
#ifdef ZEST_RING_FLAGS
        if (unit % kChunk == kChunk - kPreRead) pre_read(unit / kChunk + 1);
#endif
    }
    mutable unsigned rd_lo = 0, rd_hi = 0, rb_lo = 0, rb_hi = 0;
    mutable unsigned mc = 0;
    __device__ __forceinline__ void init_mcache(unsigned lds_addr) const {
        mc = lds_addr;
        asm volatile("" : "+v"(mc));
    }
    __device__ __forceinline__ void init_addr() const {
        const unsigned base = (unsigned)(uintptr_t)(__attribute__((address_space(3))) char *)ring;
        rd_lo = base + lane * 16, rd_hi = rd_lo + 65536, rb_lo = base + grp * 16, rb_hi = rb_lo + 65536;
        asm volatile("" : "+v"(rd_lo), "+v"(rd_hi), "+v"(rb_lo), "+v"(rb_hi));
    }
    static_assert(kRingUnits <= 128, "two 64 KiB windows");
    template <class T>
    static __device__ __forceinline__ const __attribute__((address_space(3))) T *lds_at(unsigned addr) {
        return (const __attribute__((address_space(3))) T *)(uintptr_t)addr;
    }
    __device__ __forceinline__ bf16x8 load(int unit) const {
        touch(unit);
#ifdef ZEST_EXPERIMENT_NO_LDSREAD
        const int r = unit / kChunk * kChunk % kRingUnits;
#else
        const int r = unit % kRingUnits;
#endif
        const v4u v = *lds_at<v4u>((r < 64 ? rd_lo : rd_hi) + (r % 64) * 1024);
        return *reinterpret_cast<const bf16x8 *>(&v);
    }
    __device__ __forceinline__ f32x4 load_bias(int unit, int which, int rt) const {
        if (which == 0 && rt == 0) touch(unit);
        const int r = unit % kRingUnits;
        return *lds_at<v4f>((r < 64 ? rb_lo : rb_hi) + (r % 64) * 1024 + which * 128 + rt * 64);
    }
    __device__ __forceinline__ void finish(int unit, int end) const {
#pragma unroll
        for (int u = (unit + kChunk - 1) / kChunk * kChunk; u < end; u += kChunk) {
#ifdef ZEST_RING_FLAGS
            pre_read(u / kChunk);
#endif
            enter_chunk(u / kChunk);
        }
        flush();
    }
    __device__ __forceinline__ void drain() const { asm volatile("s_waitcnt vmcnt(0)" ::: "memory"); }
};

constexpr int ep_parts(int EP) { return EP == ZEST_PREC_F16X3 ? 2 : 1; }
constexpr float kLoScale = 2048.0f, kLoUnscale = 1.0f / 2048.0f;

typedef __attribute__((ext_vector_type(2))) float f32x2_t;
typedef __attribute__((ext_vector_type(2))) __bf16 bf16x2_t;
typedef __attribute__((ext_vector_type(2))) _Float16 f16x2_t;
typedef __attribute__((ext_vector_type(8))) _Float16 f16x8_t;

template <int EP>
__device__ __forceinline__ unsigned pack_pair(float lo, float hi) {
    const f32x2_t f = {lo, hi};
    if constexpr (EP == ZEST_PREC_BF16) {
        const bf16x2_t r = __builtin_convertvector(f, bf16x2_t);
        return __builtin_bit_cast(unsigned, r);
    } else {
        const f16x2_t r = __builtin_convertvector(f, f16x2_t);
        return __builtin_bit_cast(unsigned, r);
    }
}
__device__ __forceinline__ unsigned pack_bf16(float lo, float hi) { return pack_pair<ZEST_PREC_BF16>(lo, hi); }

__device__ __forceinline__ void split_pair(float a, float b, unsigned &hi, unsigned &lo) {
    const f32x2_t f = {a, b};
    const f16x2_t h = __builtin_convertvector(f, f16x2_t);
    const f32x2_t back = __builtin_convertvector(h, f32x2_t);
    const f32x2_t rem = {(a - back[0]) * kLoScale, (b - back[1]) * kLoScale};
    const f16x2_t l = __builtin_convertvector(rem, f16x2_t);
    hi = __builtin_bit_cast(unsigned, h), lo = __builtin_bit_cast(unsigned, l);
}

template <int EP>
__device__ __forceinline__ f32x4 mfma16(bf16x8 a, bf16x8 b, f32x4 c) {
    if constexpr (EP == ZEST_PREC_BF16)
        return __builtin_amdgcn_mfma_f32_16x16x32_bf16(a, b, c, 0, 0, 0);
    else
        return __builtin_amdgcn_mfma_f32_16x16x32_f16(__builtin_bit_cast(f16x8_t, a), __builtin_bit_cast(f16x8_t, b),
                                                      c, 0, 0, 0);
}

template <int EP>
__device__ __forceinline__ float relu1(float v) {
    return __builtin_amdgcn_fmed3f(v, 0.0f, EP == ZEST_PREC_BF16 ? 3.0e38f : 65504.0f);
}

template <int N, int NP = 1>
struct OpArr {
    bf16x8 t[NP][N > 0 ? N : 1];
};

template <int EP, int N>
__device__ __forceinline__ void store_tile(const float (&v)[8], OpArr<N, ep_parts(EP)> &op, int k) {
    if constexpr (EP == ZEST_PREC_F16X3) {
        uint4 h, l;
        split_pair(v[0], v[1], h.x, l.x), split_pair(v[2], v[3], h.y, l.y);
        split_pair(v[4], v[5], h.z, l.z), split_pair(v[6], v[7], h.w, l.w);
        op.t[0][k] = __builtin_bit_cast(bf16x8, h), op.t[1][k] = __builtin_bit_cast(bf16x8, l);
    } else {
        const uint4 q = make_uint4(pack_pair<EP>(v[0], v[1]), pack_pair<EP>(v[2], v[3]), pack_pair<EP>(v[4], v[5]),
                                   pack_pair<EP>(v[6], v[7]));
        op.t[0][k] = __builtin_bit_cast(bf16x8, q);
    }
}

#ifndef ZEST_PACKED_RELU
#define ZEST_PACKED_RELU 1
#endif
typedef __attribute__((ext_vector_type(2))) short s16x2_t;
__device__ __forceinline__ unsigned relu_bf16x2(unsigned u) {
    const s16x2_t r = __builtin_elementwise_max(__builtin_bit_cast(s16x2_t, u), s16x2_t{0, 0});
    return __builtin_bit_cast(unsigned, r);
}
template <int EP, int N>
__device__ __forceinline__ void store_tile_relu16(const float (&v)[8], OpArr<N, 1> &op, int k) {
    const uint4 q = make_uint4(relu_bf16x2(pack_pair<EP>(v[0], v[1])), relu_bf16x2(pack_pair<EP>(v[2], v[3])),
                               relu_bf16x2(pack_pair<EP>(v[4], v[5])), relu_bf16x2(pack_pair<EP>(v[6], v[7])));
    op.t[0][k] = __builtin_bit_cast(bf16x8, q);
}
__device__ __forceinline__ void engine_fp16_overflow_clamp() {
    __builtin_amdgcn_s_setreg((0 << 11) | (23 << 6) | 1, 1);
}

#ifndef ZEST_PREFETCH
#define ZEST_PREFETCH 3
#endif
constexpr int kPrefetch = ZEST_PREFETCH;

#ifndef ZEST_MCACHE_JB
#define ZEST_MCACHE_JB 0
#endif
constexpr int kMcJB = ZEST_MCACHE_JB;
constexpr bool mcache_for(int EP, bool mod, int nkf) { return kMcJB > 0 && mod && nkf >= 2 && EP != ZEST_PREC_F16X3; }

template <int EP>
__device__ __forceinline__ void unpack_pairs(const v4u q, float (&v)[8]) {
#pragma unroll
    for (int i = 0; i < 4; i++) {
        if constexpr (EP == ZEST_PREC_BF16) {
            v[2 * i] = __uint_as_float(q[i] << 16), v[2 * i + 1] = __uint_as_float(q[i] & 0xFFFF0000u);
        } else {
            const f32x2_t f = __builtin_convertvector(__builtin_bit_cast(f16x2_t, q[i]), f32x2_t);
            v[2 * i] = f[0], v[2 * i + 1] = f[1];
        }
    }
}

template <int NP>
struct RowBlockPre {
    f32x4 bias[2], mbias[2];
    bf16x8 win[kPrefetch][NP];
};

struct NoSink {
    __device__ __forceinline__ void operator()(int, int, int, const float (&)[8]) const {}
};

template <int EP, int CB, int NJB, int NKA, int NKB, bool MOD, int NKF, bool RELU, int MODE, bool V2, int MC, class Tiles,
          class Sink = NoSink>
__device__ __forceinline__ void engine_layer(const Tiles &tiles, int &unit,
                                             const OpArr<NKA, ep_parts(EP)> (&opa)[CB],
                                             const OpArr<NKB, ep_parts(EP)> (&opb)[CB],
                                             const OpArr<NKF, ep_parts(EP)> (&opf)[CB],
                                             OpArr<8, ep_parts(EP)> (&out)[CB], f32x4 (&keep)[CB],
                                             int sink_id = 0, const Sink &sink = Sink()) {
    constexpr int NP = ep_parts(EP);
    constexpr bool X3 = EP == ZEST_PREC_F16X3;
    constexpr int NM = MOD ? 2 * NKF : 0, T = NM + 2 * (NKA + NKB);
    static_assert(T >= 1, "empty layer");
    constexpr bool kPackedRelu = ZEST_PACKED_RELU && RELU && MODE == 0 && EP != ZEST_PREC_F16X3 && __is_same(Sink, NoSink);
    static_assert(MC == 0 || (MOD && MODE == 0 && NJB == 8), "the modulation cache serves modulated trunk layers");
    auto k0_of = [](int jb) { return (MC == 2 && jb < kMcJB) ? NM : 0; };
    auto preload = [&](RowBlockPre<NP> &p, int u0, int k0) {
#pragma unroll
        for (int rt = 0; rt < 2; rt++) {
            p.bias[rt] = tiles.load_bias(u0, 0, rt);
            if (MOD && k0 == 0) p.mbias[rt] = tiles.load_bias(u0, 1, rt);
        }
#pragma unroll
        for (int k = 0; k < k0; k++)
#pragma unroll
            for (int pt = 0; pt < NP; pt++) tiles.touch(u0 + 1 + NP * k + pt);
#pragma unroll
        for (int k = 0; k < kPrefetch; k++)
            if (k0 + k < T) {
#pragma unroll
                for (int pt = 0; pt < NP; pt++) p.win[k][pt] = tiles.load(u0 + 1 + NP * (k0 + k) + pt);
            }
    };
    RowBlockPre<NP> pre;
    preload(pre, unit, k0_of(0));
#pragma unroll
    for (int jb = 0; jb < NJB; jb++) {
        const int u0 = unit, k0 = k0_of(jb);
        const bool mc_rd = MC == 2 && jb < kMcJB, mc_wr = MC == 1 && jb < kMcJB;
        f32x4 acc[2][CB], macc[2][CB], corr[2][CB], mcorr[2][CB];
        bf16x8 win[kPrefetch][NP];
#pragma unroll
        for (int k = 0; k < kPrefetch; k++)
#pragma unroll
            for (int pt = 0; pt < NP; pt++) win[k][pt] = pre.win[k][pt];
#pragma unroll
        for (int rt = 0; rt < 2; rt++)
#pragma unroll
            for (int cb = 0; cb < CB; cb++) {
                acc[rt][cb] = pre.bias[rt];
                if (MOD && !mc_rd) macc[rt][cb] = pre.mbias[rt];
                if (X3) corr[rt][cb] = f32x4{0.f, 0.f, 0.f, 0.f}, mcorr[rt][cb] = f32x4{0.f, 0.f, 0.f, 0.f};
            }
#pragma unroll
        for (int k = k0; k < T; k++) {
            bf16x8 a[NP];
#pragma unroll
            for (int pt = 0; pt < NP; pt++) a[pt] = win[(k - k0) % kPrefetch][pt];
            const int rt = k % 2, kt = (k < NM ? k : k - NM) / 2;
#pragma unroll
            for (int cb = 0; cb < CB; cb++) {
                auto opnd = [&](int pt) -> bf16x8 {
                    if (k < NM) return opf[cb].t[pt][k < NM ? kt : 0];
                    if (kt < NKA) return opa[cb].t[pt][(k >= NM && kt < NKA) ? kt : 0];
                    return opb[cb].t[pt][(k >= NM && kt >= NKA) ? kt - NKA : 0];
                };
                if (k < NM) {
                    macc[rt][cb] = mfma16<EP>(a[0], opnd(0), macc[rt][cb]);
                    if constexpr (X3) {
                        mcorr[rt][cb] = mfma16<EP>(a[0], opnd(NP - 1), mcorr[rt][cb]);
                        mcorr[rt][cb] = mfma16<EP>(a[NP - 1], opnd(0), mcorr[rt][cb]);
                    }
                } else {
                    acc[rt][cb] = mfma16<EP>(a[0], opnd(0), acc[rt][cb]);
                    if constexpr (X3) {
                        corr[rt][cb] = mfma16<EP>(a[0], opnd(NP - 1), corr[rt][cb]);
                        corr[rt][cb] = mfma16<EP>(a[NP - 1], opnd(0), corr[rt][cb]);
                    }
                }
            }
            if (k + kPrefetch < T) {
#pragma unroll
                for (int pt = 0; pt < NP; pt++) win[(k - k0) % kPrefetch][pt] = tiles.load(u0 + 1 + NP * (k + kPrefetch) + pt);
            }
#ifdef ZEST_SCHED_PIN
            __builtin_amdgcn_sched_barrier(0);
#endif
        }
        v4u mq[CB];
        if (mc_rd) {
#pragma unroll
            for (int cb = 0; cb < CB; cb++) mq[cb] = *Tiles::template lds_at<v4u>(tiles.mc + (jb * CB + cb) * 1024);
        }
        unit = u0 + 1 + NP * T;
        if (jb + 1 < NJB) preload(pre, unit, k0_of(jb + 1));
        tiles.flush();
#pragma unroll
        for (int cb = 0; cb < CB; cb++) {
            float v[8];
#pragma unroll
            for (int i = 0; i < 8; i++) {
                v[i] = acc[i >> 2][cb][i & 3];
                if (X3) v[i] = fmaf(corr[i >> 2][cb][i & 3], kLoUnscale, v[i]);
            }
            if (MOD) {
                float mv[8];
                if (mc_rd) {
                    unpack_pairs<EP>(mq[cb], mv);
                } else {
#pragma unroll
                    for (int i = 0; i < 8; i++) {
                        mv[i] = macc[i >> 2][cb][i & 3];
                        if (X3) mv[i] = fmaf(mcorr[i >> 2][cb][i & 3], kLoUnscale, mv[i]);
                    }
                }
                if (mc_wr) {
                    if constexpr (!X3) {
                        const uint4 q = make_uint4(pack_pair<EP>(mv[0], mv[1]), pack_pair<EP>(mv[2], mv[3]),
                                                   pack_pair<EP>(mv[4], mv[5]), pack_pair<EP>(mv[6], mv[7]));
                        *(__attribute__((address_space(3))) v4u *)(uintptr_t)(tiles.mc + (jb * CB + cb) * 1024) =
                            __builtin_bit_cast(v4u, q);
                    }
                }
#pragma unroll
                for (int i = 0; i < 8; i++) v[i] = V2 ? v[i] + mv[i] : v[i] * mv[i];
            }
            if (RELU && !kPackedRelu) {
#pragma unroll
                for (int i = 0; i < 8; i++) v[i] = relu1<EP>(v[i]);
            }
            if (MODE == 0) {
                if constexpr (kPackedRelu) store_tile_relu16<EP>(v, out[cb], jb);
                else store_tile<EP>(v, out[cb], jb);
                sink(sink_id, jb, cb, v);
            } else if (jb == 0) {
                keep[cb] = f32x4{v[0], v[1], v[2], v[3]};
            }
        }
    }
}

template <int EP, int CB, int NU_PTS, bool MOD, int NU_FEAT, bool V2, bool MCACHE = false, class Tiles, class PtsFn, class ViewsFn,
          class Sink = NoSink>
__device__ __forceinline__ void engine_forward(const Tiles &tiles, int &unit, PtsFn pts_fn,
                                               const OpArr<NU_FEAT / 2, ep_parts(EP)> (&feat)[CB], ViewsFn views_fn,
                                               f32x4 (&head)[CB], f32x4 (&rgb)[CB], const Sink &sink = Sink()) {
    constexpr int KP = NU_PTS / 2, KF = NU_FEAT / 2, NP = ep_parts(EP);
    static_assert(NU_PTS % 2 == 0 && NU_FEAT % 2 == 0, "units per row block come in row-tile pairs");
    constexpr int MC0 = (MCACHE && mcache_for(EP, MOD, KF)) ? 1 : 0, MCL = MC0 ? 2 : 0;
    OpArr<8, NP> hA[CB], hB[CB];
    OpArr<0, NP> none[CB];
    f32x4 unused[CB];
    const int unit0 = unit;
    {
        OpArr<KP, NP> pts[CB];
        pts_fn(pts, 0);
        engine_layer<EP, CB, 8, KP, 0, MOD, KF, true, 0, V2, MC0>(tiles, unit, pts, none, feat, hA, unused, 0, sink);
    }
    engine_layer<EP, CB, 8, 8, 0, MOD, KF, true, 0, V2, MCL>(tiles, unit, hA, none, feat, hB, unused, 1, sink);
    engine_layer<EP, CB, 8, 8, 0, MOD, KF, true, 0, V2, MCL>(tiles, unit, hB, none, feat, hA, unused, 2, sink);
    engine_layer<EP, CB, 8, 8, 0, MOD, KF, true, 0, V2, MCL>(tiles, unit, hA, none, feat, hB, unused, 3, sink);
    engine_layer<EP, CB, 8, 8, 0, MOD, KF, true, 0, V2, MCL>(tiles, unit, hB, none, feat, hA, unused, 4, sink);
    {
        OpArr<KP, NP> pts[CB];
        pts_fn(pts, (int)hA[CB - 1].t[0][7][0]);
        engine_layer<EP, CB, 8, KP, 8, MOD, KF, true, 0, V2, MCL>(tiles, unit, pts, hA, feat, hB, unused, 5, sink);
    }
    engine_layer<EP, CB, 8, 8, 0, MOD, KF, true, 0, V2, MCL>(tiles, unit, hB, none, feat, hA, unused, 6, sink);
    engine_layer<EP, CB, 8, 8, 0, MOD, KF, true, 0, V2, MCL>(tiles, unit, hA, none, feat, hB, unused, 7, sink);
    engine_layer<EP, CB, 1, 8, 0, false, KF, false, 1, V2, 0>(tiles, unit, hB, none, feat, hA, head);
    engine_layer<EP, CB, 8, 8, 0, false, KF, false, 0, V2, 0>(tiles, unit, hB, none, feat, hA, unused, 8, sink);
    OpArr<1, NP> views[CB];
    views_fn(views);
    engine_layer<EP, CB, 4, 8, 1, false, KF, true, 0, V2, 0>(tiles, unit, hA, views, feat, hB, unused, 9, sink);
    OpArr<4, NP> h128[CB];
#pragma unroll
    for (int cb = 0; cb < CB; cb++)
#pragma unroll
        for (int pt = 0; pt < NP; pt++)
#pragma unroll
            for (int k = 0; k < 4; k++) h128[cb].t[pt][k] = hB[cb].t[pt][k];
    engine_layer<EP, CB, 1, 4, 0, false, KF, false, 1, V2, 0>(tiles, unit, h128, none, feat, hA, rgb);
    tiles.finish(unit, unit0 + stream_units(NU_PTS, MOD ? NU_FEAT : 0, NP));
    unit = unit0 + stream_units(NU_PTS, MOD ? NU_FEAT : 0, NP);
}

int mlp_engine_launch(const MlpPlan &p, const void *tiles, const float *x, int M, float *out,
                    hipStream_t stream);

}
```

### zest-nerf_amd/csrc/mlp_engine.hip

```cpp
#include "mlp_engine.cuh"
#include "mlp_train16.h"
#include "mlp_operands.cuh"

namespace zest {

constexpr int kMlpWaves = 8;
constexpr int mlp_cb(int EP) { return EP == ZEST_PREC_F16X3 ? 1 : 2; }

__device__ __forceinline__ void stash_store(uint4 *p, uint4 q) {
#ifndef ZEST_STASH_CACHED
    __builtin_nontemporal_store(__builtin_bit_cast(v4u, q), reinterpret_cast<v4u *>(p));
#else
    *p = q;
#endif
}

template <int CB>
struct StashSink {
    uint4 *tiles;
    uint2 *masks;
    long long block;
    int lane;
    mutable unsigned lo[CB], hi[CB];
    __device__ __forceinline__ void operator()(int id, int jb, int cb, const float (&v)[8]) const {
        const int t = id < 8 ? 8 * id + jb : (id == 8 ? 64 + jb : 72 + jb);
        uint4 q = make_uint4(pack_bf16(v[0], v[1]), pack_bf16(v[2], v[3]), pack_bf16(v[4], v[5]), pack_bf16(v[6], v[7]));
        stash_store(&tiles[((block * kStashTiles + t) * CB + cb) * 64 + lane], q);
        if (id == 8) return;
        unsigned bits = 0;
#pragma unroll
        for (int i = 0; i < 8; i++) bits |= (v[i] > 0.0f ? 1u : 0u) << i;
        if (jb == 0) lo[cb] = 0, hi[cb] = 0;
        if (jb < 4) lo[cb] |= bits << (8 * jb);
        else hi[cb] |= bits << (8 * (jb - 4));
        const int last = id == 9 ? 3 : 7, mid = id == 9 ? 8 : id;
        if (jb == last) masks[((block * kStashMasks + mid) * CB + cb) * 64 + lane] = make_uint2(lo[cb], hi[cb]);
    }
};

template <int EP, int NT_PTS, bool MOD, int NT_FEAT, bool TRAIN = false, bool V2 = false>
__global__ __launch_bounds__(kMlpWaves * 64, kMlpWaves / 4) void mlp_engine_kernel(
    const uint4 *__restrict__ tiles_g, const float *__restrict__ x, int M, int P, int F, int C_in, int C_out, int head,
    int act_out, float *__restrict__ out, uint4 *__restrict__ stash_tiles = nullptr, uint2 *__restrict__ stash_masks = nullptr) {
    constexpr int NP = ep_parts(EP), CB = mlp_cb(EP), UNITS = stream_units(NT_PTS, MOD ? NT_FEAT : 0, NP);
    using Ring = RingTiles<kMlpWaves, UNITS, 0>;
    if constexpr (EP == ZEST_PREC_F16) engine_fp16_overflow_clamp();
    __shared__ __attribute__((aligned(16))) char lds[kRingUnits * 1024 + 2 * kSlots * 4];
#ifdef ZEST_RING_FLAGS
    int *ring_flags = reinterpret_cast<int *>(lds + kRingUnits * 1024);
    Ring::init_flags(ring_flags);
    __syncthreads();
#endif
    const int lane = threadIdx.x & 63, col = lane & 15, grp = lane >> 4;
    const int wave = __builtin_amdgcn_readfirstlane(threadIdx.x >> 6);
    const Ring tiles{lds, (gptr_u4)tiles_g, (gptr_u4)tiles_g, lane, grp, wave,
                     (unsigned)(wave * Ring::kPieces * 64 + lane) * 16u,
                     (unsigned)(uintptr_t)(__attribute__((address_space(3))) char *)lds +
                         (unsigned)wave * Ring::kPieces * 1024u
#ifdef ZEST_RING_FLAGS
                     , (unsigned)(uintptr_t)(__attribute__((address_space(3))) char *)ring_flags
#endif
    };
    tiles.init_addr();
    tiles.prologue();
    const int n_blocks = (M + 16 * CB - 1) / (16 * CB), n_pass = (n_blocks + kMlpWaves - 1) / kMlpWaves;
    for (int pass = blockIdx.x; pass < n_pass; pass += gridDim.x) {
        const long long m_base = ((long long)pass * kMlpWaves + wave) * (16 * CB);
        OpArr<NT_PTS / 2, NP> pts[CB];
        OpArr<NT_FEAT / 2, NP> feat[CB];
#pragma unroll
        for (int cb = 0; cb < CB; cb++) {
            const long long m = m_base + 16 * cb + col;
            const bool valid = m < M;
#ifdef ZEST_EXP_NO_XGATHER
            const float *xrow = x;
#else
            const float *xrow = x + (size_t)(valid ? m : 0) * C_in;
#endif
            load_pe_operand<EP, NT_PTS == 4 ? 3 : 4, 10, NT_PTS / 2>(xrow, valid, grp, pts[cb]);
            if (MOD) load_feat_operand<EP, NT_FEAT / 2>(xrow + P, F, valid, grp, feat[cb]);
            if constexpr (TRAIN) {
                uint4 *st = stash_tiles + (((long long)pass * kMlpWaves + wave) * kStashTiles * CB + cb) * 64 + lane;
#pragma unroll
                for (int k = 0; k < NT_PTS / 2; k++) stash_store(&st[(size_t)(kStashPts + k) * CB * 64], __builtin_bit_cast(uint4, pts[cb].t[0][k]));
                if (MOD) {
#pragma unroll
                    for (int k = 0; k < NT_FEAT / 2; k++) stash_store(&st[(size_t)(kStashFeat + k) * CB * 64], __builtin_bit_cast(uint4, feat[cb].t[0][k]));
                }
            }
        }
        auto views_fn = [&](OpArr<1, NP> (&views)[CB]) {
#pragma unroll
            for (int cb = 0; cb < CB; cb++) {
                const long long m = m_base + 16 * cb + col;
                const bool valid = m < M;
                load_pe_operand<EP, 3, 4, 1>(x + (size_t)(valid ? m : 0) * C_in + P + F, valid, grp, views[cb]);
                if constexpr (TRAIN)
                    stash_store(&stash_tiles[((((long long)pass * kMlpWaves + wave) * kStashTiles + kStashViews) * CB + cb) * 64 + lane],
                                __builtin_bit_cast(uint4, views[cb].t[0][0]));
            }
        };
        f32x4 headt[CB], rgbt[CB];
        int unit = 0;
        auto pts_fn = [&](OpArr<NT_PTS / 2, NP> (&o)[CB], int) {
#pragma unroll
            for (int cb = 0; cb < CB; cb++) o[cb] = pts[cb];
        };
        if constexpr (TRAIN) {
            const StashSink<CB> sink{stash_tiles, stash_masks, (long long)pass * kMlpWaves + wave, lane, {}, {}};
            engine_forward<EP, CB, NT_PTS, MOD, NT_FEAT, V2>(tiles, unit, pts_fn, feat, views_fn, headt, rgbt, sink);
        } else {
            engine_forward<EP, CB, NT_PTS, MOD, NT_FEAT, V2>(tiles, unit, pts_fn, feat, views_fn, headt, rgbt);
        }
#pragma unroll
        for (int cb = 0; cb < CB; cb++) {
            const long long m = m_base + 16 * cb + col;
            if (m >= M) continue;
            float *o = out + (size_t)m * C_out;
            if (grp == 0) {
                o[0] = act_out ? zest_sigmoid(rgbt[cb][0]) : rgbt[cb][0];
                o[1] = act_out ? zest_sigmoid(rgbt[cb][1]) : rgbt[cb][1];
                o[2] = act_out ? zest_sigmoid(rgbt[cb][2]) : rgbt[cb][2];
                o[3] = act_out ? fmaxf(headt[cb][0], 0.0f) : headt[cb][0];
                if (head == ZEST_HEAD_BLEND) o[4] = zest_sigmoid(headt[cb][1]);
                if (head == ZEST_HEAD_DYNAMIC)
                    o[4] = tanhf(headt[cb][1]), o[5] = tanhf(headt[cb][2]), o[6] = tanhf(headt[cb][3]);
            } else if (head == ZEST_HEAD_DYNAMIC && grp == 1) {
                o[7] = tanhf(headt[cb][0]), o[8] = tanhf(headt[cb][1]), o[9] = tanhf(headt[cb][2]);
                o[10] = zest_sigmoid(headt[cb][3]);
            } else if (head == ZEST_HEAD_DYNAMIC && grp == 2) {
                o[11] = zest_sigmoid(headt[cb][0]);
            }
        }
        tiles.next_pass();
    }
    tiles.drain();
}

template <int EP, int NT_PTS, bool MOD, int NT_FEAT, bool TRAIN = false, bool V2 = false>
static int launch_one(const MlpPlan &p, const void *tiles, const float *x, int M,
                      float *out, hipStream_t stream, void *stash_tiles = nullptr, void *stash_masks = nullptr) {
    constexpr int units = stream_units(NT_PTS, MOD ? NT_FEAT : 0, ep_parts(EP));
    if (p.n_tiles != units) {
        zest_set_error("zest_mlp_fwd(engine): plan has %d stream units, kernel expects %d", p.n_tiles, units);
        return (int)hipErrorInvalidValue;
    }
    const zest_mlp_desc &d = p.desc;
    const int F = d.use_feat ? d.in_ch_feat : 0;
    const int C_in = d.in_ch_pts + F + d.in_ch_views;
    const int C_out = d.head == ZEST_HEAD_NONE ? 4 : (d.head == ZEST_HEAD_BLEND ? 5 : 12);
    int dev = 0, cus = 256;
    if (hipGetDevice(&dev) != hipSuccess ||
        hipDeviceGetAttribute(&cus, hipDeviceAttributeMultiprocessorCount, dev) != hipSuccess)
        cus = 256;
    const int n_pass = zest_div_up(zest_div_up(M, 16 * mlp_cb(EP)), kMlpWaves);
    const int blocks = n_pass < cus ? n_pass : cus;
    if ((d.net_type >= 2) != V2) {
        zest_set_error("zest_mlp_fwd(engine): kernel / net_type mismatch");
        return (int)hipErrorInvalidValue;
    }
    hipLaunchKernelGGL((mlp_engine_kernel<EP, NT_PTS, MOD, NT_FEAT, TRAIN, V2>), dim3(blocks), dim3(kMlpWaves * 64), 0, stream,
                       (const uint4 *)tiles, x, M, d.in_ch_pts, F, C_in, C_out, d.head,
                       d.net_type == 2 ? 1 : 0, out, (uint4 *)stash_tiles, (uint2 *)stash_masks);
    ZEST_RETURN_LAUNCH(TRAIN ? "zest_mlp_train16_fwd" : "zest_mlp_fwd(engine)");
}

template <int EP>
static int launch_prec(const MlpPlan &p, const void *tiles, const float *x, int M, float *out, hipStream_t stream) {
    const bool mod = p.desc.use_feat != 0;
    const int key = p.nt_pts * 10 + (mod ? p.nt_feat : 0);
    if (p.desc.net_type >= 2) {
        switch (key) {
            case 42: return launch_one<EP, 4, true, 2, false, true>(p, tiles, x, M, out, stream);
            case 44: return launch_one<EP, 4, true, 4, false, true>(p, tiles, x, M, out, stream);
            case 62: return launch_one<EP, 6, true, 2, false, true>(p, tiles, x, M, out, stream);
            case 64: return launch_one<EP, 6, true, 4, false, true>(p, tiles, x, M, out, stream);
        }
        zest_set_error("zest_mlp_fwd(engine): no 'v2' kernel for %d point units / %d feature units per row block",
                       p.nt_pts, mod ? p.nt_feat : 0);
        return (int)hipErrorInvalidValue;
    }
    switch (key) {
        case 40: return launch_one<EP, 4, false, 0>(p, tiles, x, M, out, stream);
        case 42: return launch_one<EP, 4, true, 2>(p, tiles, x, M, out, stream);
        case 44: return launch_one<EP, 4, true, 4>(p, tiles, x, M, out, stream);
        case 60: return launch_one<EP, 6, false, 0>(p, tiles, x, M, out, stream);
        case 62: return launch_one<EP, 6, true, 2>(p, tiles, x, M, out, stream);
        case 64: return launch_one<EP, 6, true, 4>(p, tiles, x, M, out, stream);
    }
    zest_set_error("zest_mlp_fwd(engine): no kernel for %d point units / %d feature units per row "
                   "block (supported: 1..14 source views)", p.nt_pts, mod ? p.nt_feat : 0);
    return (int)hipErrorInvalidValue;
}

int mlp_engine_train_launch(const MlpPlan &p, const void *tiles, const float *x, int M, float *out, void *stash_tiles,
                            void *stash_masks, hipStream_t stream) {
    constexpr int EP = ZEST_PREC_BF16;
    const bool mod = p.desc.use_feat != 0;
    const int key = p.nt_pts * 10 + (mod ? p.nt_feat : 0);
    switch (key) {
        case 40: return launch_one<EP, 4, false, 0, true>(p, tiles, x, M, out, stream, stash_tiles, stash_masks);
        case 42: return launch_one<EP, 4, true, 2, true>(p, tiles, x, M, out, stream, stash_tiles, stash_masks);
        case 44: return launch_one<EP, 4, true, 4, true>(p, tiles, x, M, out, stream, stash_tiles, stash_masks);
        case 60: return launch_one<EP, 6, false, 0, true>(p, tiles, x, M, out, stream, stash_tiles, stash_masks);
        case 62: return launch_one<EP, 6, true, 2, true>(p, tiles, x, M, out, stream, stash_tiles, stash_masks);
        case 64: return launch_one<EP, 6, true, 4, true>(p, tiles, x, M, out, stream, stash_tiles, stash_masks);
    }
    zest_set_error("zest_mlp_train16_fwd: no kernel for %d point units / %d feature units per row block", p.nt_pts,
                   mod ? p.nt_feat : 0);
    return (int)hipErrorInvalidValue;
}

int mlp_engine_launch(const MlpPlan &p, const void *tiles, const float *x, int M, float *out,
                      hipStream_t stream) {
    switch (p.precision) {
        case ZEST_PREC_BF16: return launch_prec<ZEST_PREC_BF16>(p, tiles, x, M, out, stream);
        case ZEST_PREC_F16: return launch_prec<ZEST_PREC_F16>(p, tiles, x, M, out, stream);
        case ZEST_PREC_F16X3: return launch_prec<ZEST_PREC_F16X3>(p, tiles, x, M, out, stream);
    }
    zest_set_error("zest_mlp_fwd(engine): precision %d is not an engine operand type", p.precision);
    return (int)hipErrorInvalidValue;
}

}
```

### zest-nerf_amd/csrc/mlp_plan.h

```cpp
#pragma once
#include <stdint.h>
#include <vector>
#include "../../include/zest_render.h"

#ifdef __HIPCC__
#define ZEST_HD __host__ __device__
#else
#define ZEST_HD
#endif

namespace zest {

ZEST_HD inline int feat_volume_round(int V) { return V % 4 <= 2 ? V / 4 : V / 4 + 1; }
ZEST_HD inline int feat_quad_col(int q, int V) {
    const int r = 2 * (q >> 3) + (q & 1), g = (q & 7) >> 1, rv = feat_volume_round(V);
    if (r > rv) return -1;
    if (r == rv && g < 2) return 4 * g;
    const int view = r < rv ? 4 * r + g : 4 * rv + g - 2;
    return view < V ? 8 + 4 * view : -1;
}

constexpr int kW = 256;
constexpr int kNumOps = 12;
constexpr int kMaxSeg = 2;
constexpr int kStreamAlign = 128;

enum SlotOrder {
    ORDER_ACC = 0,
    ORDER_NATURAL = 1,
};

enum SegKind { SEG_PTS = 0, SEG_FEAT = 1, SEG_VIEWS = 2, SEG_H = 3 };

struct SegPlan {
    int kind;
    int ntiles;
};

struct OpPlan {
    int njb;
    int nseg;
    SegPlan seg[kMaxSeg];
    int mod;
    int relu;
    int tile_base;
    int tiles_per_jb;
    int bias_block;
};

struct MlpShape {
    int D, W, skip_mask;
    bool is_default;
};
bool mlp_shape(const zest_mlp_desc &d, MlpShape *s, const char **err);
void mlp_param_ld(const zest_mlp_desc &d, const MlpShape &s, int *ld);

struct MlpPlan {
    zest_mlp_desc desc;
    MlpShape shape;
    int n_ops;
    int precision, order;
    int spt;
    int ns_pts, ns_feat, ns_views;
    int nt_pts, nt_feat, nt_views, nt_h, nt_h128;
    int tail_unit0;
    int headers;
    int parts;
    int n_tiles, n_bias_blocks;
    size_t bias_bytes, bytes;
    OpPlan op[kNumOps];
    std::vector<int16_t> map_pts, map_feat, map_views;
    std::vector<uint32_t> tile_src, bias_src;
    std::vector<uint32_t> hdr_src;
    std::vector<uint8_t> unit_part;
};

inline bool prec_is_engine(int precision) {
    return precision == ZEST_PREC_BF16 || precision == ZEST_PREC_F16 || precision == ZEST_PREC_F16X3;
}

bool build_bwd_plan(const zest_mlp_desc &d, MlpPlan *out, const char **err);
constexpr int bwd_stream_units_raw(int nt_pts, int nt_feat) {
    const int kp = nt_pts / 2, mod = nt_feat;
    return 4 * (1 + 2 * 1)
           + 8 * (1 + 2 * 4)
           + 8 * (1 + mod + 2 * 9)
           + 6 * 8 * (1 + mod + 2 * 8)
           + kp * (1 + 2 * 8) + 8 * (1 + mod + 2 * 8)
           + kp * (1 + 2 * 8);
}
constexpr int bwd_stream_units(int nt_pts, int nt_feat) {
    return (bwd_stream_units_raw(nt_pts, nt_feat) + kStreamAlign - 1) / kStreamAlign * kStreamAlign;
}

struct DwJob {
    int32_t out_tile0, n_out_tiles;
    int32_t in_kind;
    int32_t in_tile0, n_in_tiles;
    int32_t ld, col0, want_bias;
    int32_t wg0, n_wg;
    int16_t out_slot[256], out_row[256];
    int16_t in_col[256];
};
constexpr int kGradTiles = 86;
constexpr int kDwStashPts = 76, kDwStashFeat = 79, kDwStashViews = 81;
int build_dw_jobs(const zest_mlp_desc &d, std::vector<DwJob> *jobs, const char **err);

bool build_plan(const zest_mlp_desc &d, int precision, int order, MlpPlan *out, const char **err,
                bool with_tables = true);

}
```

### zest-nerf_amd/csrc/mlp_plan.hip

```cpp
#include "mlp_plan.h"
#include <string.h>

namespace zest {

namespace {

inline int round_up(int a, int b) { return (a + b - 1) / b * b; }

void pe_map_acc(int C, int L, int npos, std::vector<int16_t> &m) {
    m.assign((size_t)npos, -1);
    for (int pos = 0; pos < npos; pos++) {
        const int kt = pos / 32, g = (pos % 32) / 8, e = pos % 8, mm = 8 * kt + e;
        if (mm < (L / 2) * C) {
            const int band = 2 * (mm / C) + (g >> 1), coord = mm % C;
            m[pos] = (int16_t)(C + 2 * C * band + ((g & 1) ? C : 0) + coord);
        } else if (mm == (L / 2) * C) {
            m[pos] = (int16_t)(g < C ? g : -1);
        }
    }
}

void feat_map_acc(int V, int npos, std::vector<int16_t> &m) {
    m.assign((size_t)npos, -1);
    for (int pos = 0; pos < npos; pos++) {
        const int kt = pos / 32, g = (pos % 32) / 8, e = pos % 8, q = 8 * kt + 2 * g + (e >> 2), c = e & 3;
        const int col = feat_quad_col(q, V);
        if (col >= 0) m[pos] = (int16_t)(col + c);
    }
}

void natural_map(int width, int spt, int ntiles, std::vector<int16_t> &m) {
    m.assign((size_t)ntiles * spt * 2, -1);
    for (int t = 0; t < ntiles; t++)
        for (int j = 0; j < spt; j++)
            for (int h = 0; h < 2; h++) {
                const int f = t * 2 * spt + spt * h + j;
                m[2 * (t * spt + j) + h] = (int16_t)(f < width ? f : -1);
            }
}

inline int h_feature(int order, int spt, int slot, int half) {
    if (order == ORDER_ACC) {
        const int kt = slot / 32, g = (slot % 32) / 8, e = slot % 8;
        return 32 * kt + (e < 4 ? 4 * g + e : 16 + 4 * g + (e - 4));
    }
    const int t = slot / spt, j = slot % spt;
    return t * 2 * spt + spt * half + j;
}

struct RowSrc { int param, row; };

}

bool build_plan(const zest_mlp_desc &d, int precision, int order, MlpPlan *P, const char **err,
                bool with_tables) {
    static const char *e_prec = "precision must be ZEST_PREC_F32, _BF16, _F16 or _F16X3";
    static const char *e_pts = "in_ch_pts must be 63 (xyz, L=10) or 84 (xyzt, L=10)";
    static const char *e_views = "in_ch_views must be 27 (L=4)";
    static const char *e_feat = "in_ch_feat must be 8 + 4V with 1 <= V <= 16 when use_feat is set";
    static const char *e_head = "bad head / net_type combination";
    if (precision != ZEST_PREC_F32 && !prec_is_engine(precision)) return *err = e_prec, false;
    if ((order == ORDER_ACC) != prec_is_engine(precision))
        return *err = "ORDER_ACC goes with the engine precisions, ORDER_NATURAL with fp32", false;
    if (d.in_ch_pts != 63 && d.in_ch_pts != 84) return *err = e_pts, false;
    if (d.in_ch_views != 27) return *err = e_views, false;
    const int F = d.use_feat ? d.in_ch_feat : 0;
    if (d.use_feat && (F < 12 || (F - 8) % 4 != 0 || F > 72)) return *err = e_feat, false;
    if (d.head < 0 || d.head > 2 || (d.net_type != 0 && d.net_type != 2 && d.net_type != 3) ||
        (d.net_type >= 2 && (d.head != 0 || !d.use_feat)))
        return *err = e_head, false;

    MlpShape sh;
    if (!mlp_shape(d, &sh, err)) return false;
    if (order == ORDER_ACC && !sh.is_default)
        return *err = "the MFMA engine covers depth 8 / width 256 / skips [4]; other shapes run in ZEST_PREC_F32", false;
    const int D = sh.D, Wd = sh.W;

    MlpPlan &p = *P;
    p.desc = d, p.precision = precision, p.order = order, p.shape = sh;
    p.n_ops = D + 4;
    p.spt = prec_is_engine(precision) ? 8 : 4;
    p.parts = precision == ZEST_PREC_F16X3 ? 2 : 1;
    const int spt = p.spt, C = d.in_ch_pts == 63 ? 3 : 4, V = d.use_feat ? (F - 8) / 4 : 0;
    if (order == ORDER_ACC) {
        p.ns_pts = 32 * ((5 * C + 1 + 7) / 8);
        p.ns_views = 32;
        p.ns_feat = d.use_feat ? round_up(4 * (2 + V), 32) : 0;
        pe_map_acc(C, 10, p.ns_pts, p.map_pts);
        pe_map_acc(3, 4, p.ns_views, p.map_views);
        if (d.use_feat) feat_map_acc(V, p.ns_feat, p.map_feat);
    } else {
        p.ns_pts = round_up(d.in_ch_pts, 2 * spt) / 2;
        p.ns_views = round_up(27, 2 * spt) / 2;
        p.ns_feat = d.use_feat ? round_up(F, 2 * spt) / 2 : 0;
        natural_map(d.in_ch_pts, spt, p.ns_pts / spt, p.map_pts);
        natural_map(27, spt, p.ns_views / spt, p.map_views);
        if (d.use_feat) natural_map(F, spt, p.ns_feat / spt, p.map_feat);
    }
    const int spu = order == ORDER_ACC ? 16 : spt;
    p.nt_pts = p.ns_pts / spu, p.nt_views = p.ns_views / spu, p.nt_feat = p.ns_feat / spu;
    p.nt_h = order == ORDER_ACC ? 16 : Wd / 2 / spt, p.nt_h128 = order == ORDER_ACC ? 8 : Wd / 4 / spt;

    p.headers = order == ORDER_ACC ? 1 : 0;
    memset(p.op, 0, sizeof(p.op));
    int tile = 0, bblk = d.use_feat ? Wd / 32 : 0;
    for (int o = 0; o < p.n_ops; o++) {
        OpPlan &op = p.op[o];
        op.njb = Wd / 32, op.nseg = 1, op.seg[0] = {SEG_H, p.nt_h};
        if (o < D) op.mod = d.use_feat ? 1 : 0, op.relu = 1;
        if (o == 0) op.seg[0] = {SEG_PTS, p.nt_pts};
        if (o > 0 && o < D && (sh.skip_mask >> (o - 1) & 1))
            op.nseg = 2, op.seg[0] = {SEG_PTS, p.nt_pts}, op.seg[1] = {SEG_H, p.nt_h};
        if (o == D) op.njb = 1;
        if (o == D + 2) op.njb = Wd / 64, op.relu = 1, op.nseg = 2, op.seg[1] = {SEG_VIEWS, p.nt_views};
        if (o == D + 3) op.njb = 1, op.seg[0] = {SEG_H, p.nt_h128};
        op.tiles_per_jb = (op.mod ? p.nt_feat : 0) * p.parts + p.headers;
        for (int s = 0; s < op.nseg; s++) op.tiles_per_jb += op.seg[s].ntiles * p.parts;
        op.tile_base = tile, op.bias_block = bblk;
        tile += op.njb * op.tiles_per_jb, bblk += op.njb;
    }
    if (p.headers) tile = round_up(tile, kStreamAlign), bblk = 0;
    p.n_tiles = tile, p.n_bias_blocks = bblk;
    p.bias_bytes = (size_t)round_up(bblk * 128, 1024);
    p.bytes = p.bias_bytes + (size_t)tile * 1024;

    if (!with_tables) return true;
    int ld[ZEST_P_COUNT];
    mlp_param_ld(d, sh, ld);
    const uint32_t ZERO = 0xFFFFFFFFu;
    p.tile_src.assign((size_t)tile * 64 * spt, ZERO);
    p.bias_src.assign(p.bias_bytes / 4, ZERO);
    p.hdr_src.assign(p.headers ? (size_t)tile * 64 : 0, ZERO);
    p.unit_part.assign((size_t)tile, 0);

    auto row_src = [&](int o, int row) -> RowSrc {
        if (o < D) return {ZEST_P_PTS0 + o, row};
        if (o == D + 1) return {ZEST_P_FEATURE, row};
        if (o == D + 2) return {row < Wd / 2 ? ZEST_P_VIEWS : -1, row};
        if (o == D + 3) return {row < 3 ? ZEST_P_RGB : -1, row};
        if (row == 0) return {ZEST_P_ALPHA, 0};
        if (d.head == ZEST_HEAD_BLEND && row == 1) return {ZEST_P_HEAD0, 0};
        if (d.head == ZEST_HEAD_DYNAMIC && row >= 1 && row <= 6) return {ZEST_P_HEAD0, row - 1};
        if (d.head == ZEST_HEAD_DYNAMIC && row >= 7 && row <= 8) return {ZEST_P_HEAD1, row - 7};
        return {-1, 0};
    };
    auto emit_tiles = [&](int &t, int param_of_rows_op, int jb, const SegPlan &sg, int col0,
                          bool is_mod) {
        for (int k = 0; k < sg.ntiles; k++)
          for (int part = 0; part < p.parts; part++, t++) {
            p.unit_part[t] = (uint8_t)part;
            for (int l = 0; l < 64; l++)
                for (int e = 0; e < spt; e++) {
                    int slot, half, row, feat;
                    if (order == ORDER_ACC) {
                        slot = (k / 2) * 32 + 8 * (l >> 4) + e, half = 0, row = 32 * jb + 16 * (k % 2) + (l & 15);
                        switch (sg.kind) {
                            case SEG_PTS: feat = p.map_pts[slot]; break;
                            case SEG_FEAT: feat = p.map_feat[slot]; break;
                            case SEG_VIEWS: feat = p.map_views[slot]; break;
                            default: feat = h_feature(order, spt, slot, 0);
                        }
                    } else {
                        slot = k * spt + e, half = l >> 5, row = 32 * jb + (l & 31);
                        switch (sg.kind) {
                            case SEG_PTS: feat = p.map_pts[2 * slot + half]; break;
                            case SEG_FEAT: feat = p.map_feat[2 * slot + half]; break;
                            case SEG_VIEWS: feat = p.map_views[2 * slot + half]; break;
                            default: feat = h_feature(order, spt, slot, half);
                        }
                    }
                    RowSrc rs = is_mod ? RowSrc{ZEST_P_PTS_BIAS, row} : row_src(param_of_rows_op, row);
                    if (feat < 0 || rs.param < 0) continue;
                    p.tile_src[((size_t)t * 64 + l) * spt + e] =
                        ((uint32_t)rs.param << 24) | (uint32_t)(rs.row * ld[rs.param] + col0 + feat);
                }
          }
    };
    auto emit_bias_to = [&](std::vector<uint32_t> &dst, size_t at, int o, int jb, bool is_mod) {
        for (int h = 0; h < 2; h++)
            for (int i = 0; i < 16; i++) {
                const int row = order == ORDER_ACC ? 32 * jb + 16 * h + i
                                                   : 32 * jb + (i & 3) + 8 * (i >> 2) + 4 * h;
                RowSrc rs = is_mod ? RowSrc{ZEST_P_PTS_BIAS, row} : row_src(o, row);
                if (rs.param < 0) continue;
                dst[at + h * 16 + i] = ((uint32_t)rs.param << 24) | rs.row;
            }
    };
    auto emit_bias = [&](int block, int o, int jb, bool is_mod) {
        emit_bias_to(p.bias_src, (size_t)block * 32, o, jb, is_mod);
    };
    if (d.use_feat && !p.headers)
        for (int jb = 0; jb < Wd / 32; jb++) emit_bias(jb, 0, jb, true);
    for (int o = 0; o < p.n_ops; o++) {
        const OpPlan &op = p.op[o];
        int t = op.tile_base;
        for (int jb = 0; jb < op.njb; jb++) {
            if (p.headers) {
                emit_bias_to(p.hdr_src, (size_t)t * 64, o, jb, false);
                if (op.mod) emit_bias_to(p.hdr_src, (size_t)t * 64 + 32, o, jb, true);
                t++;
            } else {
                emit_bias(op.bias_block + jb, o, jb, false);
            }
            if (op.mod) emit_tiles(t, o, jb, SegPlan{SEG_FEAT, p.nt_feat}, 0, true);
            int col0 = 0;
            for (int s = 0; s < op.nseg; s++) {
                emit_tiles(t, o, jb, op.seg[s], col0, false);
                col0 += op.seg[s].kind == SEG_PTS ? d.in_ch_pts : Wd;
            }
        }
    }
    return true;
}

bool mlp_shape(const zest_mlp_desc &d, MlpShape *s, const char **err) {
    const bool unset = d.depth == 0 && d.width == 0 && d.skip_mask == 0;
    s->D = unset ? 8 : d.depth, s->W = unset ? kW : d.width, s->skip_mask = unset ? 1 << 4 : d.skip_mask;
    if (s->D < 2 || s->D > 8) return *err = "depth must be 2 .. 8", false;
    if (s->W != 64 && s->W != 128 && s->W != 192 && s->W != 256) return *err = "width must be 64, 128, 192 or 256", false;
    if (s->skip_mask < 0 || (s->skip_mask >> (s->D - 1)) != 0) return *err = "skip_mask names a layer beyond depth", false;
    s->is_default = s->D == 8 && s->W == kW && s->skip_mask == 1 << 4;
    return true;
}

void mlp_param_ld(const zest_mlp_desc &d, const MlpShape &s, int *ld) {
    for (int l = 0; l < 8; l++)
        ld[ZEST_P_PTS0 + l] = l == 0 ? d.in_ch_pts : s.W + ((s.skip_mask >> (l - 1) & 1) ? d.in_ch_pts : 0);
    ld[ZEST_P_PTS_BIAS] = d.in_ch_feat, ld[ZEST_P_VIEWS] = s.W + d.in_ch_views, ld[ZEST_P_FEATURE] = s.W;
    ld[ZEST_P_ALPHA] = s.W, ld[ZEST_P_RGB] = s.W / 2, ld[ZEST_P_HEAD0] = s.W, ld[ZEST_P_HEAD1] = s.W;
}


namespace {

struct BwdCtx {
    const zest_mlp_desc &d;
    MlpPlan &p;
    int ld[ZEST_P_COUNT];
    int t = 0;
    std::vector<uint32_t> tile_src, hdr_src;
    void grow(int units) {
        tile_src.resize((size_t)(t + units) * 512, 0xFFFFFFFFu);
        hdr_src.resize((size_t)(t + units) * 64, 0xFFFFFFFFu);
    }
};

inline RowSrc out_row_of(const zest_mlp_desc &d, int op, int o) {
    if (op == 100) return {ZEST_P_PTS_BIAS, o};
    if (op < 8) return {ZEST_P_PTS0 + op, o};
    if (op == 9) return {ZEST_P_FEATURE, o};
    if (op == 10) return {o < kW / 2 ? ZEST_P_VIEWS : -1, o};
    if (op == 11) return {o < 3 ? ZEST_P_RGB : -1, o};
    if (o == 0) return {ZEST_P_ALPHA, 0};
    if (d.head == ZEST_HEAD_BLEND && o == 1) return {ZEST_P_HEAD0, 0};
    if (d.head == ZEST_HEAD_DYNAMIC && o >= 1 && o <= 6) return {ZEST_P_HEAD0, o - 1};
    if (d.head == ZEST_HEAD_DYNAMIC && o >= 7 && o <= 8) return {ZEST_P_HEAD1, o - 7};
    return {-1, 0};
}

template <class InCol>
void emit_bwd_row_block(BwdCtx &c, InCol in_col, int mod_jb, const int (*segs)[2], int nseg) {
    const MlpPlan &p = c.p;
    int units = 1 + (mod_jb >= 0 ? p.nt_feat : 0);
    for (int s = 0; s < nseg; s++) units += 2 * segs[s][1];
    c.grow(units);
    if (mod_jb >= 0)
        for (int i = 0; i < 32; i++)
            c.hdr_src[(size_t)c.t * 64 + 32 + i] = ((uint32_t)ZEST_P_PTS_BIAS << 24) | (uint32_t)(32 * mod_jb + i);
    c.t++;
    if (mod_jb >= 0)
        for (int k = 0; k < p.nt_feat; k++, c.t++)
            for (int l = 0; l < 64; l++)
                for (int e = 0; e < 8; e++) {
                    const int pos = (k / 2) * 32 + 8 * (l >> 4) + e, row = 32 * mod_jb + 16 * (k % 2) + (l & 15);
                    const int feat = p.map_feat[pos];
                    if (feat < 0) continue;
                    c.tile_src[((size_t)c.t * 64 + l) * 8 + e] =
                        ((uint32_t)ZEST_P_PTS_BIAS << 24) | (uint32_t)(row * c.ld[ZEST_P_PTS_BIAS] + feat);
                }
    for (int s = 0; s < nseg; s++)
        for (int k = 0; k < 2 * segs[s][1]; k++, c.t++)
            for (int l = 0; l < 64; l++)
                for (int e = 0; e < 8; e++) {
                    const int pos = (k / 2) * 32 + 8 * (l >> 4) + e;
                    const int o = h_feature(ORDER_ACC, 8, pos, 0);
                    const RowSrc rs = out_row_of(c.d, segs[s][0], o);
                    const int col = in_col(16 * (k % 2) + (l & 15));
                    if (rs.param < 0 || col < 0) continue;
                    c.tile_src[((size_t)c.t * 64 + l) * 8 + e] =
                        ((uint32_t)rs.param << 24) | (uint32_t)(rs.row * c.ld[rs.param] + col);
                }
}

}

bool build_bwd_plan(const zest_mlp_desc &d, MlpPlan *P, const char **err) {
    if (!build_plan(d, ZEST_PREC_BF16, ORDER_ACC, P, err, false)) return false;
    if (d.net_type != 0) return *err = "the bf16 training path covers 'v0' nets", false;
    MlpPlan &p = *P;
    BwdCtx c{d, p, {d.in_ch_pts, kW, kW, kW, kW, kW + d.in_ch_pts, kW, kW, d.in_ch_feat, kW + d.in_ch_views, kW, kW,
                    kW / 2, kW, kW}};
    const bool mod = d.use_feat != 0;
    const int kp = p.nt_pts / 2;
    auto natural = [](int base) { return [base](int i) { return base + i; }; };
    for (int jb = 0; jb < 4; jb++) { const int sg[1][2] = {{11, 1}}; emit_bwd_row_block(c, natural(32 * jb), -1, sg, 1); }
    for (int jb = 0; jb < 8; jb++) { const int sg[1][2] = {{10, 4}}; emit_bwd_row_block(c, natural(32 * jb), -1, sg, 1); }
    for (int jb = 0; jb < 8; jb++) { const int sg[2][2] = {{9, 8}, {8, 1}}; emit_bwd_row_block(c, natural(32 * jb), mod ? jb : -1, sg, 2); }
    for (int l = 7; l >= 1; l--) {
        const int sg[1][2] = {{l, 8}};
        if (l == 5)
            for (int jb = 0; jb < kp; jb++)
                emit_bwd_row_block(c, [&](int i) { return (int)p.map_pts[32 * jb + i]; }, -1, sg, 1);
        const int h0 = l == 5 ? d.in_ch_pts : 0;
        for (int jb = 0; jb < 8; jb++) emit_bwd_row_block(c, natural(h0 + 32 * jb), mod ? jb : -1, sg, 1);
    }
    for (int jb = 0; jb < kp; jb++) {
        const int sg[1][2] = {{0, 8}};
        emit_bwd_row_block(c, [&](int i) { return (int)p.map_pts[32 * jb + i]; }, -1, sg, 1);
    }
    if (c.t != bwd_stream_units_raw(p.nt_pts, mod ? p.nt_feat : 0)) return *err = "backward stream: unit count mismatch", false;
    int total = round_up(c.t, kStreamAlign);
    c.grow(total - c.t);
    c.t = total;
    p.tail_unit0 = total;
    if (mod) {
        for (int jb = 0; jb < p.nt_feat / 2; jb++) {
            const int sg[1][2] = {{100, 8}};
            emit_bwd_row_block(c, [&](int i) { return (int)p.map_feat[32 * jb + i]; }, -1, sg, 1);
        }
        for (int jb = 0; jb < 8; jb++) emit_bwd_row_block(c, [](int) { return -1; }, jb, nullptr, 0);
    }
    total = c.t;
    p.headers = 1, p.parts = 1, p.n_tiles = total, p.n_bias_blocks = 0, p.bias_bytes = 0;
    p.bytes = (size_t)total * 1024;
    p.tile_src.swap(c.tile_src), p.hdr_src.swap(c.hdr_src);
    p.bias_src.clear();
    p.unit_part.assign((size_t)total, 0);
    return true;
}

int build_dw_jobs(const zest_mlp_desc &d, std::vector<DwJob> *jobs, const char **err) {
    MlpPlan p;
    if (!build_plan(d, ZEST_PREC_BF16, ORDER_ACC, &p, err, false)) return -1;
    jobs->clear();
    const bool mod = d.use_feat != 0;
    const int kp = p.nt_pts / 2, kf = p.nt_feat / 2;
    auto add = [&](int op, int out_tile0, int n_out, int in_kind, int in_tile0, int n_in, int ld, int col0, int bias,
                   const std::vector<int16_t> *in_map) {
        DwJob j;
        memset(&j, 0, sizeof(j));
        j.out_tile0 = out_tile0, j.n_out_tiles = n_out, j.in_kind = in_kind, j.in_tile0 = in_tile0, j.n_in_tiles = n_in;
        j.ld = ld, j.col0 = col0, j.want_bias = bias;
        for (int pos = 0; pos < 256; pos++) {
            j.out_slot[pos] = -1, j.out_row[pos] = 0, j.in_col[pos] = -1;
            if (pos < 32 * n_out) {
                const int o = h_feature(ORDER_ACC, 8, pos, 0);
                const RowSrc rs = out_row_of(d, op, o);
                j.out_slot[pos] = (int16_t)rs.param, j.out_row[pos] = (int16_t)rs.row;
            }
            if (pos < 32 * n_in)
                j.in_col[pos] = in_map ? (*in_map)[pos] : (int16_t)h_feature(ORDER_ACC, 8, pos, 0);
        }
        jobs->push_back(j);
    };
    for (int l = 0; l < 8; l++) {
        const int ld = l == 0 ? d.in_ch_pts : (l == 5 ? kW + d.in_ch_pts : kW);
        if (l == 0 || l == 5) add(l, 8 * l, 8, 1, kDwStashPts, kp, ld, 0, l == 0, &p.map_pts);
        if (l > 0) add(l, 8 * l, 8, 0, 8 * (l - 1), 8, ld, l == 5 ? d.in_ch_pts : 0, 1, nullptr);
    }
    add(8, 76, 1, 0, 56, 8, kW, 0, 1, nullptr);
    add(9, 64, 8, 0, 56, 8, kW, 0, 1, nullptr);
    add(10, 72, 4, 0, 64, 8, kW + d.in_ch_views, 0, 1, nullptr);
    add(10, 72, 4, 3, kDwStashViews, 1, kW + d.in_ch_views, kW, 0, &p.map_views);
    add(11, 77, 1, 0, 72, 4, kW / 2, 0, 1, nullptr);
    if (mod) add(100, 78, 8, 2, kDwStashFeat, kf, d.in_ch_feat, 0, 1, &p.map_feat);
    return (int)jobs->size();
}

}
```

Before: 9.706 million rays/s.

## Fold feature linear layer into views layer weights for inference streams

Result: faster. 10.77 million rays/s, median of 6 (+10.9%).

```diff
diff --git a/zest-nerf_amd/csrc/fused.cuh b/zest-nerf_amd/csrc/fused.cuh
--- a/zest-nerf_amd/csrc/fused.cuh
+++ b/zest-nerf_amd/csrc/fused.cuh
@@ -315,7 +315,7 @@
     constexpr bool MOD_S = NT_FEAT_S > 0, MOD_D = NT_FEAT_D > 0;
     constexpr int NP = ep_parts(EP), CB = fused_cb(EP), BS = 16 * CB;
     if constexpr (EP == ZEST_PREC_F16) engine_fp16_overflow_clamp();
-    constexpr int UNITS_S = stream_units(4, NT_FEAT_S, NP), UNITS_D = DYN ? stream_units(6, NT_FEAT_D, NP) : 0;
+    constexpr int UNITS_S = stream_units(4, NT_FEAT_S, NP, true), UNITS_D = DYN ? stream_units(6, NT_FEAT_D, NP, true) : 0;
     using Ring = RingTiles<kFusedWaves, UNITS_S, UNITS_D>;
     constexpr int kFdBytes = (DYN && MOD_D && ZEST_EARLY_DYN_GATHER) ? kFusedWaves * CB * (NT_FEAT_D / 2) * NP * 1024 : 0;
     constexpr int kStBytes = DYN ? kFusedWaves * 32 * 24 : 0;
@@ -488,7 +488,7 @@
         };
         ZEST_STAMP(st_enc);
         if constexpr (ZEST_REBUILD_PTS) {
-            engine_forward<EP, CB, 4, MOD_S, NT_FEAT_S, V2S, true>(tiles, unit, pts_static, feat_s,
+            engine_forward<EP, CB, 4, MOD_S, NT_FEAT_S, V2S, true, true>(tiles, unit, pts_static, feat_s,
                                                         views_of(a.st, cams_s), head_s, rgb_s);
         } else {
             OpArr<2, NP> pts_keep[CB];
@@ -497,7 +497,7 @@
 #pragma unroll
                 for (int cb = 0; cb < CB; cb++) o[cb] = pts_keep[cb];
             };
-            engine_forward<EP, CB, 4, MOD_S, NT_FEAT_S, V2S, true>(tiles, unit, pts_copy, feat_s,
+            engine_forward<EP, CB, 4, MOD_S, NT_FEAT_S, V2S, true, true>(tiles, unit, pts_copy, feat_s,
                                                         views_of(a.st, cams_s), head_s, rgb_s);
         }
         ZEST_STAMP(st_eng);
@@ -549,7 +549,7 @@
             }
             ZEST_STAMP(st_comp);
             if constexpr (ZEST_REBUILD_PTS) {
-                engine_forward<EP, CB, 6, MOD_D, NT_FEAT_D, false, true>(tiles, unit, pts_dynamic, feat_d,
+                engine_forward<EP, CB, 6, MOD_D, NT_FEAT_D, false, true, true>(tiles, unit, pts_dynamic, feat_d,
                                                             views_of(a.dy, cams_d), head_d, rgb_d);
             } else {
                 OpArr<3, NP> pts_keep[CB];
@@ -558,7 +558,7 @@
 #pragma unroll
                     for (int cb = 0; cb < CB; cb++) o[cb] = pts_keep[cb];
                 };
-                engine_forward<EP, CB, 6, MOD_D, NT_FEAT_D, false, true>(tiles, unit, pts_copy, feat_d,
+                engine_forward<EP, CB, 6, MOD_D, NT_FEAT_D, false, true, true>(tiles, unit, pts_copy, feat_d,
                                                             views_of(a.dy, cams_d), head_d, rgb_d);
             }
             ZEST_STAMP(st_eng);
@@ -634,7 +634,7 @@
         ZEST_RETURN_LAUNCH("zest_render_fused_fwd(" #ptag "_" #tag ")");                         \
     }                                                                                            \
     int fused_units_##ptag##_##tag(int which) {                                                  \
-        return which == 0 ? stream_units(4, NTS, ep_parts(EP)) : (DYN ? stream_units(6, NTD, ep_parts(EP)) : 0); \
+        return which == 0 ? stream_units(4, NTS, ep_parts(EP), true) : (DYN ? stream_units(6, NTD, ep_parts(EP), true) : 0); \
     }
 
 #define ZEST_FUSED_DECL1(ptag, tag)                                                     \
diff --git a/zest-nerf_amd/csrc/fused.hip b/zest-nerf_amd/csrc/fused.hip
--- a/zest-nerf_amd/csrc/fused.hip
+++ b/zest-nerf_amd/csrc/fused.hip
@@ -23,9 +23,9 @@
     if (d->in_ch_pts != pts_ch) return *err = "unexpected in_ch_pts for this slot", false;
     if (d->net_type != 0 && d->net_type != 2) return *err = "net_type must be 0 ('v0') or 2 ('v2')", false;
     zest::MlpPlan plan;
-    if (!zest::build_plan(*d, precision, zest::ORDER_ACC, &plan, err, false)) return false;
-    n->bias = (const float *)packed;
-    n->tiles = (const uint4 *)((const char *)packed + plan.bias_bytes);
+    if (!zest::build_plan(*d, precision, zest::ORDER_ACC, &plan, err, false, true)) return false;
+    n->bias = (const float *)((const char *)packed + plan.stream_off);
+    n->tiles = (const uint4 *)((const char *)n->bias + plan.bias_bytes);
     n->head = d->head, n->v2 = d->net_type == 2;
     *nt_feat = d->use_feat ? plan.nt_feat : 0;
     *units = plan.n_tiles;
diff --git a/zest-nerf_amd/csrc/mlp.hip b/zest-nerf_amd/csrc/mlp.hip
--- a/zest-nerf_amd/csrc/mlp.hip
+++ b/zest-nerf_amd/csrc/mlp.hip
@@ -20,6 +20,7 @@
 std::map<std::tuple<int, int, int, int, int, int, int, int, int, int, int, int>, DevPlan *> g_plans;
 
 constexpr int kOrderBwd = 99;
+constexpr int kOrderFold = 98;
 
 DevPlan *get_plan(const zest_mlp_desc &d, int precision, int order, bool need_tables) {
     int dev = 0;
@@ -32,8 +33,9 @@
     if (!dp) {
         dp = new DevPlan();
         const char *err = nullptr;
-        const bool ok = order == kOrderBwd ? zest::build_bwd_plan(d, &dp->plan, &err)
-                                           : zest::build_plan(d, precision, order, &dp->plan, &err);
+        const bool ok = order == kOrderBwd    ? zest::build_bwd_plan(d, &dp->plan, &err)
+                        : order == kOrderFold ? zest::build_plan(d, precision, zest::ORDER_ACC, &dp->plan, &err, true, true)
+                                              : zest::build_plan(d, precision, order, &dp->plan, &err);
         if (!ok) {
             zest_set_error("MLP shape not supported: %s", err);
             delete dp;
@@ -66,8 +68,27 @@
 }
 
 struct ParamTable {
-    const float *p[2 * ZEST_P_COUNT];
+    const float *p[2 * zest::kParamSlots];
 };
+
+__global__ __launch_bounds__(zest::kW) void fold_view_kernel(const float *__restrict__ wv, const float *__restrict__ bv,
+                                                             const float *__restrict__ wf, const float *__restrict__ bf,
+                                                             int ld_v, float *__restrict__ wc, float *__restrict__ bc) {
+    constexpr int W = zest::kW;
+    const int r = blockIdx.x, c = threadIdx.x;
+    if (r < W / 2) {
+        double acc = 0.0;
+        for (int k = 0; k < W; k++) acc += (double)wv[(size_t)r * ld_v + k] * (double)wf[(size_t)k * W + c];
+        wc[(size_t)r * W + c] = (float)acc;
+    } else if (c < W / 2) {
+        double acc = 0.0;
+        for (int k = 0; k < W; k++) acc += (double)wv[(size_t)c * ld_v + k] * (double)bf[k];
+        bc[c] = (float)(acc + (double)bv[c]);
+    } else {
+        bc[c] = 0.0f;
+    }
+}
+static_assert(zest::kFoldScratchBytes == zest::kFoldBiasOffset + (size_t)zest::kW * 4, "bc [W/2] and W/2 floats of padding");
 
 template <int PREC>
 __global__ void pack_kernel(ParamTable pt, const uint32_t *__restrict__ tile_src, size_t n_w,
@@ -245,7 +266,7 @@
     DevPlan *dp = get_plan(d, ZEST_PREC_BF16, kOrderBwd, true);
     if (!dp) return (int)hipErrorInvalidValue;
     const MlpPlan &p = dp->plan;
-    ParamTable pt;
+    ParamTable pt = {};
     for (int i = 0; i < 2 * ZEST_P_COUNT; i++) pt.p[i] = params[i];
     const size_t n_w = p.tile_src.size(), n_h = p.hdr_src.size();
     hipLaunchKernelGGL(pack_kernel<ZEST_PREC_BF16>, dim3(zest_div_up(n_w, 256)), dim3(256), 0, stream, pt, dp->tile_src,
@@ -258,6 +279,10 @@
 
 extern "C" size_t zest_mlp_packed_bytes(const zest_mlp_desc *desc, int precision) {
     if (!desc) return 0;
+    if (zest::prec_is_engine(precision)) {
+        DevPlan *df = get_plan(*desc, precision, kOrderFold, false);
+        return df ? df->plan.stream_off + df->plan.bytes : 0;
+    }
     DevPlan *dp = get_plan(*desc, precision, order_for(precision), false);
     return dp ? dp->plan.bytes : 0;
 }
@@ -268,7 +293,9 @@
     DevPlan *dp = get_plan(*desc, precision, order_for(precision), true);
     if (!dp) return (int)hipErrorInvalidValue;
     const MlpPlan &p = dp->plan;
-    ParamTable pt;
+    DevPlan *df = zest::prec_is_engine(precision) ? get_plan(*desc, precision, kOrderFold, true) : nullptr;
+    if (zest::prec_is_engine(precision) && !df) return (int)hipErrorInvalidValue;
+    ParamTable pt = {};
     for (int i = 0; i < 2 * ZEST_P_COUNT; i++) pt.p[i] = params[i];
     bool need[ZEST_P_COUNT] = {};
     for (int i = 0; i < p.shape.D; i++) need[i] = true;
@@ -280,24 +307,36 @@
         ZEST_CHECK_ARG(!need[i] || (params[2 * i] && params[2 * i + 1]),
                        "zest_mlp_pack: parameter slot %d (weight and bias) is required", i);
     ZEST_CHECK_ARG(((uintptr_t)packed & 15) == 0, "zest_mlp_pack: packed must be 16-byte aligned");
-    const size_t n_w = p.tile_src.size(), n_b = p.bias_src.size();
-    const size_t n = n_w > n_b ? n_w : n_b;
-    void *w_out = (char *)packed + p.bias_bytes;
+    auto pack_stream = [&](const DevPlan *q, char *base) {
+        const size_t n_w = q->plan.tile_src.size(), n_b = q->plan.bias_src.size();
+        const size_t n = n_w > n_b ? n_w : n_b;
+        void *w_out = base + q->plan.bias_bytes;
 #define ZEST_PACK(PREC)                                                                            \
     hipLaunchKernelGGL(pack_kernel<PREC>, dim3(zest_div_up(n, 256)), dim3(256), 0, (hipStream_t)stream, \
-                       pt, dp->tile_src, n_w, dp->bias_src, n_b, dp->unit_part, (float *)packed, w_out)
-    if (zest::prec_is_engine(precision)) {
-        if (precision == ZEST_PREC_BF16) ZEST_PACK(ZEST_PREC_BF16);
-        else if (precision == ZEST_PREC_F16) ZEST_PACK(ZEST_PREC_F16);
-        else ZEST_PACK(ZEST_PREC_F16X3);
-        const size_t n_h = p.hdr_src.size();
-        if (n_h)
-            hipLaunchKernelGGL(pack_headers_kernel, dim3(zest_div_up(n_h, 256)), dim3(256), 0,
-                               (hipStream_t)stream, pt, dp->hdr_src, n_h, (char *)w_out);
-    } else {
-        ZEST_PACK(ZEST_PREC_F32);
-    }
+                       pt, q->tile_src, n_w, q->bias_src, n_b, q->unit_part, (float *)base, w_out)
+        if (zest::prec_is_engine(precision)) {
+            if (precision == ZEST_PREC_BF16) ZEST_PACK(ZEST_PREC_BF16);
+            else if (precision == ZEST_PREC_F16) ZEST_PACK(ZEST_PREC_F16);
+            else ZEST_PACK(ZEST_PREC_F16X3);
+            const size_t n_h = q->plan.hdr_src.size();
+            if (n_h)
+                hipLaunchKernelGGL(pack_headers_kernel, dim3(zest_div_up(n_h, 256)), dim3(256), 0,
+                                   (hipStream_t)stream, pt, q->hdr_src, n_h, (char *)w_out);
+        } else {
+            ZEST_PACK(ZEST_PREC_F32);
+        }
 #undef ZEST_PACK
+    };
+    pack_stream(dp, (char *)packed);
+    if (df) {
+        float *wc = (float *)((char *)packed + zest::fold_scratch_offset(p.bytes));
+        float *bc = (float *)((char *)wc + zest::kFoldBiasOffset);
+        hipLaunchKernelGGL(fold_view_kernel, dim3(zest::kW / 2 + 1), dim3(zest::kW), 0, (hipStream_t)stream,
+                           params[2 * ZEST_P_VIEWS], params[2 * ZEST_P_VIEWS + 1], params[2 * ZEST_P_FEATURE],
+                           params[2 * ZEST_P_FEATURE + 1], zest::kW + desc->in_ch_views, wc, bc);
+        pt.p[2 * zest::kFoldSlot] = wc, pt.p[2 * zest::kFoldSlot + 1] = bc;
+        pack_stream(df, (char *)packed + df->plan.stream_off);
+    }
     ZEST_RETURN_LAUNCH("zest_mlp_pack");
 }
 
@@ -306,12 +345,12 @@
     if (M == 0) return 0;
     ZEST_CHECK_ARG(desc && packed && x && out, "zest_mlp_fwd: null argument");
     ZEST_CHECK_ARG(M >= 0, "zest_mlp_fwd: M=%d", M);
-    DevPlan *dp = get_plan(*desc, precision, order_for(precision), false);
+    DevPlan *dp = get_plan(*desc, precision, zest::prec_is_engine(precision) ? kOrderFold : order_for(precision), false);
     if (!dp) return (int)hipErrorInvalidValue;
     if (M == 0) return 0;
     const MlpPlan &p = dp->plan;
-    const float *bias = (const float *)packed;
-    const void *tiles = (const char *)packed + p.bias_bytes;
+    const float *bias = (const float *)((const char *)packed + p.stream_off);
+    const void *tiles = (const char *)bias + p.bias_bytes;
     if (precision == ZEST_PREC_F32) {
         const F32Prog pr = make_f32_prog(p);
         const size_t lds = (size_t)(pr.rows_pts + pr.rows_feat + 32 + 2 * pr.W) * 32 * sizeof(float);
diff --git a/zest-nerf_amd/csrc/mlp_engine.cuh b/zest-nerf_amd/csrc/mlp_engine.cuh
--- a/zest-nerf_amd/csrc/mlp_engine.cuh
+++ b/zest-nerf_amd/csrc/mlp_engine.cuh
@@ -13,14 +13,16 @@
 
 namespace zest {
 
-constexpr int stream_units_raw(int nt_pts, int nt_feat, int parts = 1) {
+constexpr int stream_units_raw(int nt_pts, int nt_feat, int parts = 1, bool fold = false) {
     const int mod = nt_feat * parts, P = nt_pts * parts, H = 16 * parts;
     return 8 * (1 + mod + P) + 6 * 8 * (1 + mod + H) + 8 * (1 + mod + P + H)
-           + (1 + H) + 8 * (1 + H) + 4 * (1 + H + 2 * parts) + (1 + H / 2);
-}
-constexpr int stream_units(int nt_pts, int nt_feat, int parts = 1) {
-    return (stream_units_raw(nt_pts, nt_feat, parts) + kStreamAlign - 1) / kStreamAlign * kStreamAlign;
-}
+           + (1 + H) + (fold ? 0 : 8 * (1 + H)) + 4 * (1 + H + 2 * parts) + (1 + H / 2);
+}
+constexpr int stream_units(int nt_pts, int nt_feat, int parts = 1, bool fold = false) {
+    return (stream_units_raw(nt_pts, nt_feat, parts, fold) + kStreamAlign - 1) / kStreamAlign * kStreamAlign;
+}
+static_assert(stream_units_raw(4, 0) == 1262 && stream_units_raw(4, 0, 1, true) == 1126 &&
+              stream_units(4, 0, 1, true) == 9 * kStreamAlign, "unit counts of the headline net (DESIGN.md 3.1)");
 
 #ifndef ZEST_CHUNK
 #define ZEST_CHUNK 16
@@ -517,8 +519,8 @@
     }
 }
 
-template <int EP, int CB, int NU_PTS, bool MOD, int NU_FEAT, bool V2, bool MCACHE = false, class Tiles, class PtsFn, class ViewsFn,
-          class Sink = NoSink>
+template <int EP, int CB, int NU_PTS, bool MOD, int NU_FEAT, bool V2, bool MCACHE = false, bool FOLD = false, class Tiles,
+          class PtsFn, class ViewsFn, class Sink = NoSink>
 __device__ __forceinline__ void engine_forward(const Tiles &tiles, int &unit, PtsFn pts_fn,
                                                const OpArr<NU_FEAT / 2, ep_parts(EP)> (&feat)[CB], ViewsFn views_fn,
                                                f32x4 (&head)[CB], f32x4 (&rgb)[CB], const Sink &sink = Sink()) {
@@ -546,20 +548,22 @@
     engine_layer<EP, CB, 8, 8, 0, MOD, KF, true, 0, V2, MCL>(tiles, unit, hB, none, feat, hA, unused, 6, sink);
     engine_layer<EP, CB, 8, 8, 0, MOD, KF, true, 0, V2, MCL>(tiles, unit, hA, none, feat, hB, unused, 7, sink);
     engine_layer<EP, CB, 1, 8, 0, false, KF, false, 1, V2, 0>(tiles, unit, hB, none, feat, hA, head);
-    engine_layer<EP, CB, 8, 8, 0, false, KF, false, 0, V2, 0>(tiles, unit, hB, none, feat, hA, unused, 8, sink);
+    if constexpr (!FOLD)
+        engine_layer<EP, CB, 8, 8, 0, false, KF, false, 0, V2, 0>(tiles, unit, hB, none, feat, hA, unused, 8, sink);
+    OpArr<8, NP> (&vin)[CB] = FOLD ? hB : hA, (&vout)[CB] = FOLD ? hA : hB;
     OpArr<1, NP> views[CB];
     views_fn(views);
-    engine_layer<EP, CB, 4, 8, 1, false, KF, true, 0, V2, 0>(tiles, unit, hA, views, feat, hB, unused, 9, sink);
+    engine_layer<EP, CB, 4, 8, 1, false, KF, true, 0, V2, 0>(tiles, unit, vin, views, feat, vout, unused, 9, sink);
     OpArr<4, NP> h128[CB];
 #pragma unroll
     for (int cb = 0; cb < CB; cb++)
 #pragma unroll
         for (int pt = 0; pt < NP; pt++)
 #pragma unroll
-            for (int k = 0; k < 4; k++) h128[cb].t[pt][k] = hB[cb].t[pt][k];
-    engine_layer<EP, CB, 1, 4, 0, false, KF, false, 1, V2, 0>(tiles, unit, h128, none, feat, hA, rgb);
-    tiles.finish(unit, unit0 + stream_units(NU_PTS, MOD ? NU_FEAT : 0, NP));
-    unit = unit0 + stream_units(NU_PTS, MOD ? NU_FEAT : 0, NP);
+            for (int k = 0; k < 4; k++) h128[cb].t[pt][k] = vout[cb].t[pt][k];
+    engine_layer<EP, CB, 1, 4, 0, false, KF, false, 1, V2, 0>(tiles, unit, h128, none, feat, vin, rgb);
+    tiles.finish(unit, unit0 + stream_units(NU_PTS, MOD ? NU_FEAT : 0, NP, FOLD));
+    unit = unit0 + stream_units(NU_PTS, MOD ? NU_FEAT : 0, NP, FOLD);
 }
 
 int mlp_engine_launch(const MlpPlan &p, const void *tiles, const float *x, int M, float *out,
diff --git a/zest-nerf_amd/csrc/mlp_engine.hip b/zest-nerf_amd/csrc/mlp_engine.hip
--- a/zest-nerf_amd/csrc/mlp_engine.hip
+++ b/zest-nerf_amd/csrc/mlp_engine.hip
@@ -42,7 +42,8 @@
 __global__ __launch_bounds__(kMlpWaves * 64, kMlpWaves / 4) void mlp_engine_kernel(
     const uint4 *__restrict__ tiles_g, const float *__restrict__ x, int M, int P, int F, int C_in, int C_out, int head,
     int act_out, float *__restrict__ out, uint4 *__restrict__ stash_tiles = nullptr, uint2 *__restrict__ stash_masks = nullptr) {
-    constexpr int NP = ep_parts(EP), CB = mlp_cb(EP), UNITS = stream_units(NT_PTS, MOD ? NT_FEAT : 0, NP);
+    constexpr bool FOLD = !TRAIN;
+    constexpr int NP = ep_parts(EP), CB = mlp_cb(EP), UNITS = stream_units(NT_PTS, MOD ? NT_FEAT : 0, NP, FOLD);
     using Ring = RingTiles<kMlpWaves, UNITS, 0>;
     if constexpr (EP == ZEST_PREC_F16) engine_fp16_overflow_clamp();
     __shared__ __attribute__((aligned(16))) char lds[kRingUnits * 1024 + 2 * kSlots * 4];
@@ -108,9 +109,9 @@
         };
         if constexpr (TRAIN) {
             const StashSink<CB> sink{stash_tiles, stash_masks, (long long)pass * kMlpWaves + wave, lane, {}, {}};
-            engine_forward<EP, CB, NT_PTS, MOD, NT_FEAT, V2>(tiles, unit, pts_fn, feat, views_fn, headt, rgbt, sink);
+            engine_forward<EP, CB, NT_PTS, MOD, NT_FEAT, V2, false, false>(tiles, unit, pts_fn, feat, views_fn, headt, rgbt, sink);
         } else {
-            engine_forward<EP, CB, NT_PTS, MOD, NT_FEAT, V2>(tiles, unit, pts_fn, feat, views_fn, headt, rgbt);
+            engine_forward<EP, CB, NT_PTS, MOD, NT_FEAT, V2, false, true>(tiles, unit, pts_fn, feat, views_fn, headt, rgbt);
         }
 #pragma unroll
         for (int cb = 0; cb < CB; cb++) {
@@ -140,9 +141,10 @@
 template <int EP, int NT_PTS, bool MOD, int NT_FEAT, bool TRAIN = false, bool V2 = false>
 static int launch_one(const MlpPlan &p, const void *tiles, const float *x, int M,
                       float *out, hipStream_t stream, void *stash_tiles = nullptr, void *stash_masks = nullptr) {
-    constexpr int units = stream_units(NT_PTS, MOD ? NT_FEAT : 0, ep_parts(EP));
-    if (p.n_tiles != units) {
-        zest_set_error("zest_mlp_fwd(engine): plan has %d stream units, kernel expects %d", p.n_tiles, units);
+    constexpr int units = stream_units(NT_PTS, MOD ? NT_FEAT : 0, ep_parts(EP), !TRAIN);
+    if (p.n_tiles != units || (p.fold != 0) != !TRAIN) {
+        zest_set_error("zest_mlp_fwd(engine): plan has %d stream units (fold %d), kernel expects %d (fold %d)", p.n_tiles,
+                       p.fold, units, TRAIN ? 0 : 1);
         return (int)hipErrorInvalidValue;
     }
     const zest_mlp_desc &d = p.desc;
diff --git a/zest-nerf_amd/csrc/mlp_plan.h b/zest-nerf_amd/csrc/mlp_plan.h
--- a/zest-nerf_amd/csrc/mlp_plan.h
+++ b/zest-nerf_amd/csrc/mlp_plan.h
@@ -24,6 +24,13 @@
 constexpr int kNumOps = 12;
 constexpr int kMaxSeg = 2;
 constexpr int kStreamAlign = 128;
+
+constexpr int kFoldSlot = ZEST_P_COUNT;
+constexpr int kParamSlots = ZEST_P_COUNT + 1;
+constexpr size_t kFoldBiasOffset = (size_t)(kW / 2) * kW * 4;
+constexpr size_t kFoldScratchBytes = (kFoldBiasOffset + (size_t)(kW / 2) * 4 + 1023) / 1024 * 1024;
+constexpr size_t fold_scratch_offset(size_t plain_bytes) { return plain_bytes; }
+constexpr size_t infer_stream_offset(size_t plain_bytes) { return plain_bytes + kFoldScratchBytes; }
 
 enum SlotOrder {
     ORDER_ACC = 0,
@@ -66,6 +73,8 @@
     int tail_unit0;
     int headers;
     int parts;
+    int fold;
+    size_t stream_off;
     int n_tiles, n_bias_blocks;
     size_t bias_bytes, bytes;
     OpPlan op[kNumOps];
@@ -107,6 +116,6 @@
 int build_dw_jobs(const zest_mlp_desc &d, std::vector<DwJob> *jobs, const char **err);
 
 bool build_plan(const zest_mlp_desc &d, int precision, int order, MlpPlan *out, const char **err,
-                bool with_tables = true);
+                bool with_tables = true, bool fold = false);
 
 }
diff --git a/zest-nerf_amd/csrc/mlp_plan.hip b/zest-nerf_amd/csrc/mlp_plan.hip
--- a/zest-nerf_amd/csrc/mlp_plan.hip
+++ b/zest-nerf_amd/csrc/mlp_plan.hip
@@ -53,7 +53,7 @@
 }
 
 bool build_plan(const zest_mlp_desc &d, int precision, int order, MlpPlan *P, const char **err,
-                bool with_tables) {
+                bool with_tables, bool fold) {
     static const char *e_prec = "precision must be ZEST_PREC_F32, _BF16, _F16 or _F16X3";
     static const char *e_pts = "in_ch_pts must be 63 (xyz, L=10) or 84 (xyzt, L=10)";
     static const char *e_views = "in_ch_views must be 27 (L=4)";
@@ -62,6 +62,7 @@
     if (precision != ZEST_PREC_F32 && !prec_is_engine(precision)) return *err = e_prec, false;
     if ((order == ORDER_ACC) != prec_is_engine(precision))
         return *err = "ORDER_ACC goes with the engine precisions, ORDER_NATURAL with fp32", false;
+    if (fold && order != ORDER_ACC) return *err = "only the engine's stream (ORDER_ACC) has a folded form", false;
     if (d.in_ch_pts != 63 && d.in_ch_pts != 84) return *err = e_pts, false;
     if (d.in_ch_views != 27) return *err = e_views, false;
     const int F = d.use_feat ? d.in_ch_feat : 0;
@@ -81,6 +82,7 @@
     p.n_ops = D + 4;
     p.spt = prec_is_engine(precision) ? 8 : 4;
     p.parts = precision == ZEST_PREC_F16X3 ? 2 : 1;
+    p.fold = fold ? 1 : 0, p.stream_off = 0;
     const int spt = p.spt, C = d.in_ch_pts == 63 ? 3 : 4, V = d.use_feat ? (F - 8) / 4 : 0;
     if (order == ORDER_ACC) {
         p.ns_pts = 32 * ((5 * C + 1 + 7) / 8);
@@ -112,6 +114,7 @@
         if (o > 0 && o < D && (sh.skip_mask >> (o - 1) & 1))
             op.nseg = 2, op.seg[0] = {SEG_PTS, p.nt_pts}, op.seg[1] = {SEG_H, p.nt_h};
         if (o == D) op.njb = 1;
+        if (o == D + 1 && fold) op.njb = 0;
         if (o == D + 2) op.njb = Wd / 64, op.relu = 1, op.nseg = 2, op.seg[1] = {SEG_VIEWS, p.nt_views};
         if (o == D + 3) op.njb = 1, op.seg[0] = {SEG_H, p.nt_h128};
         op.tiles_per_jb = (op.mod ? p.nt_feat : 0) * p.parts + p.headers;
@@ -123,6 +126,11 @@
     p.n_tiles = tile, p.n_bias_blocks = bblk;
     p.bias_bytes = (size_t)round_up(bblk * 128, 1024);
     p.bytes = p.bias_bytes + (size_t)tile * 1024;
+    if (fold) {
+        MlpPlan plain;
+        if (!build_plan(d, precision, order, &plain, err, false, false)) return false;
+        p.stream_off = infer_stream_offset(plain.bytes);
+    }
 
     if (!with_tables) return true;
     int ld[ZEST_P_COUNT];
@@ -136,7 +144,7 @@
     auto row_src = [&](int o, int row) -> RowSrc {
         if (o < D) return {ZEST_P_PTS0 + o, row};
         if (o == D + 1) return {ZEST_P_FEATURE, row};
-        if (o == D + 2) return {row < Wd / 2 ? ZEST_P_VIEWS : -1, row};
+        if (o == D + 2) return {row < Wd / 2 ? (fold ? kFoldSlot : ZEST_P_VIEWS) : -1, row};
         if (o == D + 3) return {row < 3 ? ZEST_P_RGB : -1, row};
         if (row == 0) return {ZEST_P_ALPHA, 0};
         if (d.head == ZEST_HEAD_BLEND && row == 1) return {ZEST_P_HEAD0, 0};
@@ -171,8 +179,11 @@
                     }
                     RowSrc rs = is_mod ? RowSrc{ZEST_P_PTS_BIAS, row} : row_src(param_of_rows_op, row);
                     if (feat < 0 || rs.param < 0) continue;
+                    const bool folded_h = rs.param == kFoldSlot && sg.kind == SEG_H;
+                    const int param = rs.param == kFoldSlot && !folded_h ? (int)ZEST_P_VIEWS : rs.param;
+                    const int ldp = folded_h ? Wd : ld[param];
                     p.tile_src[((size_t)t * 64 + l) * spt + e] =
-                        ((uint32_t)rs.param << 24) | (uint32_t)(rs.row * ld[rs.param] + col0 + feat);
+                        ((uint32_t)param << 24) | (uint32_t)(rs.row * ldp + col0 + feat);
                 }
           }
     };
```
